# MLCogUP/nspeech

Hardware: AMD Instinct MI355X
Metric: mel-frames/sec Tacotron-2 LJSpeech bs32 train step (higher is better)
Workload: dtype bf16; 1 GPU; Tacotron-2 train step (fwd+bwd+clip+Adam), batch 32/GPU, T_in 160, T_out 1000, r=5; targets = spectrogram features of synthetic speech (SURVEY 8d); global_batch=32, parallelism=dp1, deterministic_gradients=True

## Files before the change

nspeech_amd/csrc/lstm_cluster.hip:

```cpp
#include "common.h"
#include <stdlib.h>
#include <stdint.h>

typedef unsigned long long u64;
constexpr int CW = 8;
constexpr int CTHREADS = CW * 64;

struct LstmClusterArgs {
  int N, T, H, P, padl, CS;
  const float* xg[2]; long ld_xg;
  const bf16_t* whT[2];
  const bf16_t* wh[2];
  bf16_t* h[2]; long ld_h;
  float* c[2];
  bf16_t* gates[2];
  const bf16_t* whT_hi[2]; const bf16_t* whT_lo[2];
  float* hf[2]; bf16_t* hb[2]; long ld_hb;
  const float* dh[2]; long ld_dh;
  bf16_t* dgates[2];
  const int* lengths;
  float forget_bias, cell_clip;
  u64* xbuf;
  int* status;
  int dbg;
  unsigned* flags;
  long long* trace;
};

__device__ __forceinline__ int swz_off(int row, int k, int H) {
  const int chunk = k >> 3;
  const int m = ((H >> 3) & 15) ? 7 : 15;
  return row * H + (((chunk ^ (row & m)) << 3) | (k & 7));
}

__global__ __launch_bounds__(CTHREADS) void lstm_cluster_fwd_kernel(LstmClusterArgs a) {
  extern __shared__ __attribute__((aligned(16))) char smem[];
  bf16_t* hs = (bf16_t*)smem;
  const int tid = threadIdx.x, lane = tid & 63, wave = tid >> 6;
  const int CS = a.CS, H = a.H;
  const int nrg = (a.N + 15) / 16;
  const int chain = blockIdx.x / CS, wgc = blockIdx.x % CS;
  const int d = chain / nrg, rg = chain % nrg;
  const int n0 = rg * 16;
  const int r16 = lane & 15, g = lane >> 4;
  const int GPR = H / 2;
  u64* xb = a.xbuf + (size_t)chain * 2 * 16 * GPR;
  const int uw0 = wgc * 64 + wave * 8;
  const int ksteps = H / 32;

  bf16x8 bw[2][16];
  {
    const bf16_t* W = a.whT[d];
    const int unit = uw0 + (r16 & 7);
#pragma unroll
    for (int tl = 0; tl < 2; ++tl) {
      const int gate = tl * 2 + (r16 >> 3);
      const bf16_t* row = W + ((long)gate * H + unit) * H;
#pragma unroll
      for (int ks = 0; ks < 16; ++ks)
        bw[tl][ks] = ks < ksteps ? *(const bf16x8*)(row + ks * 32 + g * 8) : (bf16x8){0, 0, 0, 0, 0, 0, 0, 0};
    }
  }
  float cst[4] = {0.f, 0.f, 0.f, 0.f};
  const bool cell_lane = r16 < 8;
  const int unit = uw0 + (r16 & 7);
  int len[4];
#pragma unroll
  for (int r = 0; r < 4; ++r) {
    const int n = n0 + g * 4 + r;
    len[r] = (a.lengths && n < a.N) ? a.lengths[n] : a.T;
  }
  const float* xg = a.xg[d];
  float xa[4], xb2[4], xa_n[4], xb_n[4];
  auto load_xg = [&](int t, float* pa, float* pb) {
#pragma unroll
    for (int r = 0; r < 4; ++r) {
      const int n = n0 + g * 4 + r;
      const long rowi = (long)n * a.P + a.padl + t;
      const bool ok = n < a.N;
      const int ga = (r16 >> 3), gb = 2 + (r16 >> 3);
      pa[r] = (ok && !(a.dbg & 1)) ? xg[rowi * a.ld_xg + (long)ga * H + unit] : 0.f;
      pb[r] = (ok && !(a.dbg & 1)) ? xg[rowi * a.ld_xg + (long)gb * H + unit] : 0.f;
    }
  };
  load_xg(d ? a.T - 1 : 0, xa, xb2);

  for (int step = 0; step < a.T; ++step) {
    const int t = d ? a.T - 1 - step : step;
    if (step + 1 < a.T) load_xg(d ? t - 1 : t + 1, xa_n, xb_n);
    f32x4 accA = {xa[0], xa[1], xa[2], xa[3]};
    f32x4 accB = {xb2[0], xb2[1], xb2[2], xb2[3]};
    if (step > 0) {
      const u64* cur = xb + (size_t)(step & 1) * 16 * GPR;
      const int total = 16 * GPR;
      for (int i0 = tid; i0 < total; i0 += CTHREADS * 4) {
        u64 v[4];
        unsigned spins = 0, clk0 = 0;
        bool ok;
        do {
          ok = true;
#pragma unroll
          for (int j = 0; j < 4; ++j) {
            const int i = i0 + j * CTHREADS;
            v[j] = i < total ? __hip_atomic_load(cur + i, __ATOMIC_RELAXED, __HIP_MEMORY_SCOPE_AGENT)
                             : ((u64)(unsigned)step << 32);
          }
#pragma unroll
          for (int j = 0; j < 4; ++j) ok = ok && ((unsigned)(v[j] >> 32) == (unsigned)step);
          if (a.dbg & 4) ok = true;
          if (!ok && (++spins & 1023u) == 0 && ns_spin_timed_out(clk0)) { atomicExch(a.status, 1); ok = true; }
        } while (!ok);
#pragma unroll
        for (int j = 0; j < 4; ++j) {
          const int i = i0 + j * CTHREADS;
          if (i < total) {
            const int row = i / GPR, pr = i % GPR;
            *(unsigned*)(hs + swz_off(row, pr * 2, H)) = (unsigned)v[j];
          }
        }
      }
      __syncthreads();
      if (*(volatile int*)a.status) return;
#pragma unroll
      for (int ks = 0; ks < 16; ++ks) {
        if (ks < ksteps) {
          const bf16x8 af = *(const bf16x8*)(hs + swz_off(r16, ks * 32 + g * 8, H));
          accA = __builtin_amdgcn_mfma_f32_16x16x32_bf16(af, bw[0][ks], accA, 0, 0, 0);
          accB = __builtin_amdgcn_mfma_f32_16x16x32_bf16(af, bw[1][ks], accB, 0, 0, 0);
        }
      }
      __syncthreads();
    }
    float hv[4], sgi[4], sgj[4], sgf[4], sgo[4];
#pragma unroll
    for (int r = 0; r < 4; ++r) {
      const float zj = __shfl_down(accA[r], 8, 64);
      const float zo = __shfl_down(accB[r], 8, 64);
      const bool masked = t >= len[r];
      const float gi = sigmoidf_(accA[r]), gj = tanhf_(zj), gf = sigmoidf_(accB[r] + a.forget_bias), go = sigmoidf_(zo);
      float cn = ns_cell_clip(gf * cst[r] + gi * gj, a.cell_clip);
      float hn = go * tanhf_(cn);
      if (masked) { cn = 0.f; hn = 0.f; }
      cst[r] = cn;
      hv[r] = hn;
      sgi[r] = masked ? 0.f : gi; sgj[r] = masked ? 0.f : gj; sgf[r] = masked ? 0.f : gf; sgo[r] = masked ? 0.f : go;
    }
    if (step + 1 < a.T) {
      u64* nxt = xb + (size_t)((step + 1) & 1) * 16 * GPR;
#pragma unroll
      for (int r = 0; r < 4; ++r) {
        const float hp = __shfl_down(hv[r], 1, 64);
        if (cell_lane && !(r16 & 1)) {
          const bf16_t b0 = (bf16_t)hv[r], b1 = (bf16_t)hp;
          const unsigned pay = (unsigned)(*(const unsigned short*)&b0) | ((unsigned)(*(const unsigned short*)&b1) << 16);
          const int row = g * 4 + r;
          __hip_atomic_store(nxt + (size_t)row * GPR + (unit >> 1), ((u64)(unsigned)(step + 1) << 32) | pay,
                             __ATOMIC_RELAXED, __HIP_MEMORY_SCOPE_AGENT);
        }
      }
    }
#pragma unroll
    for (int r = 0; r < 4; ++r) {
      const int n = n0 + g * 4 + r;
      if (cell_lane && n < a.N && !(a.dbg & 2)) {
        const long rowi = (long)n * a.P + a.padl + t;
        a.h[d][rowi * a.ld_h + unit] = (bf16_t)hv[r];
        a.c[d][rowi * H + unit] = cst[r];
        bf16_t* gp = a.gates[d] + rowi * 4 * H;
        gp[unit] = (bf16_t)sgi[r];
        gp[H + unit] = (bf16_t)sgj[r];
        gp[2 * H + unit] = (bf16_t)sgf[r];
        gp[3 * H + unit] = (bf16_t)sgo[r];
      }
    }
#pragma unroll
    for (int r = 0; r < 4; ++r) { xa[r] = xa_n[r]; xb2[r] = xb_n[r]; }
  }
}

__global__ __launch_bounds__(CTHREADS) void lstm_cluster_bwd_kernel(LstmClusterArgs a) {
  extern __shared__ __attribute__((aligned(16))) char smem[];
  const int CS = a.CS, H = a.H, K = 4 * a.H;
  bf16_t* dgs = (bf16_t*)smem;
  float* red = (float*)(smem + (size_t)16 * K * 2);
  const int tid = threadIdx.x, lane = tid & 63, wave = tid >> 6;
  const int nrg = (a.N + 15) / 16;
  const int chain = blockIdx.x / CS, wgc = blockIdx.x % CS;
  const int d = chain / nrg, rg = chain % nrg;
  const int n0 = rg * 16;
  const int r16 = lane & 15, g = lane >> 4;
  const int GPR = K / 2;
  u64* xb = a.xbuf + (size_t)chain * 2 * 16 * GPR;
  const int u0 = wgc * 64;
  const int kpw = K / CW;
  const int ksteps = kpw / 32;
  bf16x8 bw[4][8];
  {
    const bf16_t* W = a.wh[d];
#pragma unroll
    for (int tl = 0; tl < 4; ++tl) {
      const bf16_t* row = W + (long)(u0 + tl * 16 + r16) * K + wave * kpw;
#pragma unroll
      for (int ks = 0; ks < 8; ++ks)
        bw[tl][ks] = ks < ksteps ? *(const bf16x8*)(row + ks * 32 + g * 8) : (bf16x8){0, 0, 0, 0, 0, 0, 0, 0};
    }
  }
  const int er = tid >> 5, eu = (tid & 31) * 2;
  const int en = n0 + er;
  const int elen = (a.lengths && en < a.N) ? a.lengths[en] : a.T;
  float dcc[2] = {0.f, 0.f};

  for (int step = a.T - 1; step >= 0; --step) {
    const int t = d ? a.T - 1 - step : step;
    const int tp = d ? t + 1 : t - 1;
    const bool has_prev = step > 0;
    const bool has_next = step < a.T - 1;
    const int bs = a.T - 1 - step;
    float pdh[2] = {0.f, 0.f}, pg[2][4], pc[2] = {0.f, 0.f}, pcp[2] = {0.f, 0.f};
    const long rowi = (long)en * a.P + a.padl + t;
    const bool ok = en < a.N;
    const bool masked = t >= elen;
#pragma unroll
    for (int q = 0; q < 2; ++q) {
      const int u = u0 + eu + q;
#pragma unroll
      for (int j = 0; j < 4; ++j) pg[q][j] = ok ? (float)a.gates[d][rowi * 4 * H + (long)j * H + u] : 0.f;
      if (ok) {
        pdh[q] = a.dh[d][rowi * a.ld_dh + u];
        pc[q] = a.c[d][rowi * H + u];
        if (has_prev) pcp[q] = a.c[d][((long)en * a.P + a.padl + tp) * H + u];
      }
    }
    float dhp[2] = {0.f, 0.f};
    if (has_next) {
      const u64* cur = xb + (size_t)(bs & 1) * 16 * GPR;
      const int total = 16 * GPR;
      for (int i0 = tid; i0 < total; i0 += CTHREADS * 8) {
        u64 v[8];
        unsigned spins = 0, clk0 = 0;
        bool okk;
        do {
          okk = true;
#pragma unroll
          for (int j = 0; j < 8; ++j) {
            const int i = i0 + j * CTHREADS;
            v[j] = i < total ? __hip_atomic_load(cur + i, __ATOMIC_RELAXED, __HIP_MEMORY_SCOPE_AGENT)
                             : ((u64)(unsigned)bs << 32);
          }
#pragma unroll
          for (int j = 0; j < 8; ++j) okk = okk && ((unsigned)(v[j] >> 32) == (unsigned)bs);
          if (!okk && (++spins & 1023u) == 0 && ns_spin_timed_out(clk0)) { atomicExch(a.status, 2); okk = true; }
        } while (!okk);
#pragma unroll
        for (int j = 0; j < 8; ++j) {
          const int i = i0 + j * CTHREADS;
          if (i < total) {
            const int row = i / GPR, pr = i % GPR;
            *(unsigned*)(dgs + swz_off(row, pr * 2, K)) = (unsigned)v[j];
          }
        }
      }
      __syncthreads();
      if (*(volatile int*)a.status) return;
      f32x4 acc[4];
#pragma unroll
      for (int tl = 0; tl < 4; ++tl) acc[tl] = (f32x4){0.f, 0.f, 0.f, 0.f};
#pragma unroll
      for (int ks = 0; ks < 8; ++ks) {
        if (ks < ksteps) {
          const bf16x8 af = *(const bf16x8*)(dgs + swz_off(r16, wave * kpw + ks * 32 + g * 8, K));
#pragma unroll
          for (int tl = 0; tl < 4; ++tl) acc[tl] = __builtin_amdgcn_mfma_f32_16x16x32_bf16(af, bw[tl][ks], acc[tl], 0, 0, 0);
        }
      }
#pragma unroll
      for (int tl = 0; tl < 4; ++tl)
#pragma unroll
        for (int r = 0; r < 4; ++r) red[(wave * 16 + g * 4 + r) * 65 + tl * 16 + r16] = acc[tl][r];
      __syncthreads();
#pragma unroll
      for (int q = 0; q < 2; ++q) {
        float s = 0.f;
#pragma unroll
        for (int w = 0; w < CW; ++w) s += red[(w * 16 + er) * 65 + eu + q];
        dhp[q] = s;
      }
    }
    float dgv[2][4];
#pragma unroll
    for (int q = 0; q < 2; ++q) {
      const float gi = pg[q][0], gj = pg[q][1], gf = pg[q][2], go = pg[q][3];
      const float dh = pdh[q] + dhp[q];
      const float tc = tanhf_(pc[q]);
      const float d_o = dh * tc * go * (1.f - go);
      const float dc = dh * go * (1.f - tc * tc) + dcc[q];
      dgv[q][0] = dc * gj * gi * (1.f - gi);
      dgv[q][1] = dc * gi * (1.f - gj * gj);
      dgv[q][2] = dc * pcp[q] * gf * (1.f - gf);
      dgv[q][3] = d_o;
      dcc[q] = dc * gf;
      if (masked || !ok) {
        dgv[q][0] = dgv[q][1] = dgv[q][2] = dgv[q][3] = 0.f;
        dcc[q] = 0.f;
      }
    }
    if (step > 0) {
      u64* nxt = xb + (size_t)((bs + 1) & 1) * 16 * GPR;
#pragma unroll
      for (int j = 0; j < 4; ++j) {
        const bf16_t b0 = (bf16_t)dgv[0][j], b1 = (bf16_t)dgv[1][j];
        const unsigned pay = (unsigned)(*(const unsigned short*)&b0) | ((unsigned)(*(const unsigned short*)&b1) << 16);
        __hip_atomic_store(nxt + (size_t)er * GPR + ((j * H + u0 + eu) >> 1), ((u64)(unsigned)(bs + 1) << 32) | pay,
                           __ATOMIC_RELAXED, __HIP_MEMORY_SCOPE_AGENT);
      }
    }
    if (ok) {
#pragma unroll
      for (int j = 0; j < 4; ++j) {
        const bf16_t b0 = (bf16_t)dgv[0][j], b1 = (bf16_t)dgv[1][j];
        const unsigned pay = (unsigned)(*(const unsigned short*)&b0) | ((unsigned)(*(const unsigned short*)&b1) << 16);
        *(unsigned*)(a.dgates[d] + rowi * 4 * H + (long)j * H + u0 + eu) = pay;
      }
    }
    __syncthreads();
  }
}

constexpr int XW = 4;
constexpr int FW_POLL = 2;
constexpr int FW_WAVES = XW + 2 + FW_POLL;
constexpr int BW_POLL = 2;
constexpr int BW_WAVES = XW + 1 + BW_POLL + 1;
constexpr int XG_LD = 256 + 4;

__device__ __forceinline__ void wg_barrier() { asm volatile("s_waitcnt lgkmcnt(0)\n\ts_barrier" ::: "memory"); }
__device__ __forceinline__ unsigned pack_bf16(float lo, float hi) {
  const bf16_t b0 = (bf16_t)lo, b1 = (bf16_t)hi;
  return (unsigned)(*(const unsigned short*)&b0) | ((unsigned)(*(const unsigned short*)&b1) << 16);
}

template <int HB, int R>
__global__ __launch_bounds__(FW_WAVES * 64) void lstm_cluster2_fwd_kernel(LstmClusterArgs a) {
  extern __shared__ __attribute__((aligned(16))) char smem[];
  constexpr int H = HB * 64, KS = H / 32, CS = HB;
  constexpr int GPD = XW * 64 * 2;
  bf16_t* hs = (bf16_t*)smem;
  float* xgs = (float*)(smem + (size_t)2 * 16 * H * 2);
  constexpr int SV_H = 16 * 64 * 2, SV_C = 16 * 64 * 4, SV_G = 16 * 4 * 64 * 2, SV_BYTES = SV_H + SV_C + SV_G;
  char* svs = (char*)(xgs + 2 * 16 * XG_LD);
  int* abortf = (int*)(svs + 2 * SV_BYTES);
  const int tid = threadIdx.x, lane = tid & 63;
  const int wave = __builtin_amdgcn_readfirstlane(tid >> 6);
  const int nsets = ((a.N + 15) / 16 + R - 1) / R;
  const int set = blockIdx.x / CS, wgc = blockIdx.x % CS;
  const int d = set / nsets, rg0 = (set % nsets) * R;
  const int r16 = lane & 15, g = lane >> 4;
  u64* xb0 = a.xbuf + (size_t)(d * nsets * R + rg0) * 2 * CS * GPD;
  const int u0 = wgc * 64;
  const int T = a.T, Q = a.T * R;
  if (tid < 3) abortf[tid] = 0;

  if (wave < XW) {
    const int wq = wave * 16 + g * 4;
    bf16x8 bw[4][KS];
    {
      const bf16_t* W = a.whT[d];
#pragma unroll
      for (int gate = 0; gate < 4; ++gate) {
        const bf16_t* row = W + ((long)gate * H + u0 + wave * 16 + r16) * H;
#pragma unroll
        for (int ks = 0; ks < KS; ++ks) bw[gate][ks] = *(const bf16x8*)(row + ks * 32 + g * 8);
      }
    }
    float cst[R][4];
    int len[R];
    uint2 pend[R];
#pragma unroll
    for (int rg = 0; rg < R; ++rg) {
      const int n = (rg0 + rg) * 16 + r16;
      len[rg] = (a.lengths && n < a.N) ? a.lengths[n] : T;
      pend[rg] = make_uint2(0u, 0u);
#pragma unroll
      for (int r = 0; r < 4; ++r) cst[rg][r] = 0.f;
    }
    f32x4 acc[4];
    auto load_xg = [&](int q) {
      const float* xr = xgs + ((size_t)(q & 1) * 16 + r16) * XG_LD + wq;
#pragma unroll
      for (int gate = 0; gate < 4; ++gate) acc[gate] = *(const f32x4*)(xr + gate * 64);
    };
    wg_barrier();
    load_xg(0);
    for (int step = 0; step < T; ++step) {
      const int t = d ? T - 1 - step : step;
#pragma unroll
      for (int rg = 0; rg < R; ++rg) {
        const int q = step * R + rg, buf = q & 1;
        wg_barrier();
        if (abortf[buf]) return;
        const bool tr = (a.dbg & 16) && blockIdx.x == 0 && tid == 0 && q < 512;
        if (tr) a.trace[q * 8 + 0] = wall_clock64();
        if (R == 2 && q > 0)
          *(uint2*)(hs + (size_t)((q + 1) & 1) * 16 * H + swz_off(r16, u0 + wq, H)) = pend[(rg + 1) % R];
        if (step > 0) {
          const bf16_t* hb = hs + (size_t)buf * 16 * H;
#pragma unroll
          for (int ks = 0; ks < KS; ++ks) {
            const bf16x8 hf = *(const bf16x8*)(hb + swz_off(r16, ks * 32 + g * 8, H));
#pragma unroll
            for (int gate = 0; gate < 4; ++gate)
              acc[gate] = __builtin_amdgcn_mfma_f32_16x16x32_bf16(bw[gate][ks], hf, acc[gate], 0, 0, 0);
          }
        }
        const bool masked = t >= len[rg];
        float hv[4], sg[4][4];
#pragma unroll
        for (int r = 0; r < 4; ++r) {
          const float gi = sigmoidf_(acc[0][r]), gj = tanhf_(acc[1][r]);
          const float gf = sigmoidf_(acc[2][r] + a.forget_bias), go = sigmoidf_(acc[3][r]);
          float cn = ns_cell_clip(gf * cst[rg][r] + gi * gj, a.cell_clip);
          float hn = go * tanhf_(cn);
          if (masked) { cn = 0.f; hn = 0.f; }
          cst[rg][r] = cn;
          hv[r] = hn;
          sg[r][0] = masked ? 0.f : gi; sg[r][1] = masked ? 0.f : gj; sg[r][2] = masked ? 0.f : gf; sg[r][3] = masked ? 0.f : go;
        }
        if (tr) a.trace[q * 8 + 1] = wall_clock64();
        uint2 hp;
        hp.x = pack_bf16(hv[0], hv[1]);
        hp.y = pack_bf16(hv[2], hv[3]);
        if (step + 1 < T) {
          if (CS > 1) {
            u64* nxt = xb0 + ((size_t)rg * 2 + ((step + 1) & 1)) * CS * GPD + (size_t)wgc * GPD + (wave * 64 + lane) * 2;
            __hip_atomic_store(nxt, ((u64)(unsigned)(step + 1) << 32) | hp.x, __ATOMIC_RELAXED, __HIP_MEMORY_SCOPE_AGENT);
            __hip_atomic_store(nxt + 1, ((u64)(unsigned)(step + 1) << 32) | hp.y, __ATOMIC_RELAXED, __HIP_MEMORY_SCOPE_AGENT);
          }
          if (R == 1) *(uint2*)(hs + (size_t)((q + 1) & 1) * 16 * H + swz_off(r16, u0 + wq, H)) = hp;
          else pend[rg] = hp;
        }
        if (tr) a.trace[q * 8 + 2] = wall_clock64();
        {
          char* sv = svs + (size_t)buf * SV_BYTES;
          *(uint2*)((bf16_t*)sv + r16 * 64 + wq) = hp;
          *(f32x4*)((float*)(sv + SV_H) + r16 * 64 + wq) = (f32x4){cst[rg][0], cst[rg][1], cst[rg][2], cst[rg][3]};
          bf16_t* gp = (bf16_t*)(sv + SV_H + SV_C) + r16 * 4 * 64 + wq;
#pragma unroll
          for (int gate = 0; gate < 4; ++gate) {
            uint2 pk;
            pk.x = pack_bf16(sg[0][gate], sg[1][gate]);
            pk.y = pack_bf16(sg[2][gate], sg[3][gate]);
            *(uint2*)(gp + gate * 64) = pk;
          }
        }
        if (q + 1 < Q) load_xg(q + 1);
      }
    }
    wg_barrier();
  } else if (wave == XW || wave == XW + 3) {
    constexpr int NPG = (CS - 1) * GPD;
    constexpr int PPG = NPG / (FW_POLL * 64) > 0 ? NPG / (FW_POLL * 64) : 1;
    static_assert(CS == 1 || NPG == PPG * FW_POLL * 64, "poller coverage");
    const int j0 = (wave == XW ? 0 : 1) * PPG;
    wg_barrier();
    for (int q = 0; q < Q; ++q) {
      const int step = q / R, rg = q % R, buf = q & 1;
      const bool tr = (a.dbg & 16) && blockIdx.x == 0 && lane == 0 && wave == XW && q < 512;
      if (tr) a.trace[q * 8 + 4] = wall_clock64();
      if (step > 0 && CS > 1) {
        const u64* cur = xb0 + ((size_t)rg * 2 + (step & 1)) * CS * GPD;
        u64 v[PPG];
        unsigned spins = 0, clk0 = 0;
        bool ok;
        do {
          ok = true;
#pragma unroll
          for (int j = 0; j < PPG; ++j) {
            const int li = lane + 64 * (j0 + j), sx = li / GPD;
            const int ws = sx < wgc ? sx : sx + 1;
            v[j] = __hip_atomic_load(cur + (size_t)ws * GPD + (li % GPD), __ATOMIC_RELAXED, __HIP_MEMORY_SCOPE_AGENT);
          }
#pragma unroll
          for (int j = 0; j < PPG; ++j) ok = ok && ((unsigned)(v[j] >> 32) == (unsigned)step);
          if (!ok) {
            if ((++spins & 1023u) == 0) {
              if (__hip_atomic_load(a.status, __ATOMIC_RELAXED, __HIP_MEMORY_SCOPE_AGENT)) { abortf[buf] = 1; ok = true; }
              else if (ns_spin_timed_out(clk0)) { atomicExch(a.status, 1); abortf[buf] = 1; ok = true; }
            }
          }
        } while (!ok);
        if (tr) { a.trace[q * 8 + 5] = wall_clock64(); a.trace[q * 8 + 6] = spins; }
        bf16_t* dst = hs + (size_t)buf * 16 * H;
#pragma unroll
        for (int j = 0; j < PPG; ++j) {
          const int li = lane + 64 * (j0 + j), sx = li / GPD, lw = li % GPD;
          const int ws = sx < wgc ? sx : sx + 1;
          const int lp = (lw >> 1) & 63;
          const int k = ws * 64 + (lw >> 7) * 16 + (lp >> 4) * 4 + (lw & 1) * 2;
          *(unsigned*)(dst + swz_off(lp & 15, k, H)) = (unsigned)v[j];
        }
      }
      wg_barrier();
      if (abortf[buf]) return;
    }
    wg_barrier();
  } else if (wave == XW + 2) {
    auto save = [&](int q) {
      const int step = q / R, rg = q % R;
      const int t = d ? T - 1 - step : step;
      const int n0 = (rg0 + rg) * 16;
      const char* sv = svs + (size_t)(q & 1) * SV_BYTES;
#pragma unroll
      for (int j = 0; j < 14; ++j) {
        const int idx = lane + 64 * j;
        const f32x4 v = *(const f32x4*)(sv + idx * 16);
        if (idx < 128) {
          const int row = idx >> 3, cc = idx & 7;
          if (n0 + row < a.N)
            *(f32x4*)(a.h[d] + ((unsigned)((n0 + row) * a.P + a.padl + t) * (unsigned)a.ld_h + (unsigned)(u0 + cc * 8))) = v;
        } else if (idx < 384) {
          const int jj = idx - 128, row = jj >> 4, cc = jj & 15;
          if (n0 + row < a.N)
            *(f32x4*)(a.c[d] + ((unsigned)((n0 + row) * a.P + a.padl + t) * (unsigned)H + (unsigned)(u0 + cc * 4))) = v;
        } else {
          const int jj = idx - 384, row = jj >> 5, gate = (jj >> 3) & 3, cc = jj & 7;
          if (n0 + row < a.N)
            *(f32x4*)(a.gates[d] + ((unsigned)((n0 + row) * a.P + a.padl + t) * (unsigned)(4 * H) + (unsigned)(gate * H + u0 + cc * 8))) = v;
        }
      }
    };
    wg_barrier();
    for (int q = 0; q < Q; ++q) {
      wg_barrier();
      if (abortf[q & 1]) return;
      if (q > 0) save(q - 1);
    }
    wg_barrier();
    save(Q - 1);
  } else {
    f32x4 pf[16];
    const float* xg = a.xg[d];
    const int pgate = lane >> 4, pf4 = (lane & 15) * 4;
    auto pf_load = [&](int q) {
      const int step = q / R, rg = q % R;
      const int t = d ? T - 1 - step : step;
      const int n0 = (rg0 + rg) * 16;
#pragma unroll
      for (int j = 0; j < 16; ++j) {
        const int n = n0 + j;
        pf[j] = n < a.N ? *(const f32x4*)(xg + ((unsigned)(n * a.P + a.padl + t) * (unsigned)a.ld_xg + (unsigned)(pgate * H + u0 + pf4)))
                        : (f32x4){0.f, 0.f, 0.f, 0.f};
      }
    };
    auto pf_store = [&](int buf) {
#pragma unroll
      for (int j = 0; j < 16; ++j) *(f32x4*)(xgs + ((size_t)buf * 16 + j) * XG_LD + pgate * 64 + pf4) = pf[j];
    };
    pf_load(0);
    pf_store(0);
    if (Q > 1) pf_load(1);
    wg_barrier();
    for (int q = 0; q < Q; ++q) {
      if (q + 1 < Q) {
        pf_store((q + 1) & 1);
        if (q + 2 < Q) pf_load(q + 2);
      }
      wg_barrier();
      if (abortf[q & 1]) return;
    }
    wg_barrier();
  }
}


constexpr int X3W = 4, X3_POLL = 2, X3_UPW = 32;
constexpr int X3_WAVES = X3W + X3_POLL + 2;
constexpr int XG3_LD = 4 * X3_UPW + 4;

template <int HB, int R>
__global__ __launch_bounds__(X3_WAVES * 64) void lstm_cluster3_fwd_kernel(LstmClusterArgs a) {
  extern __shared__ __attribute__((aligned(16))) char smem[];
  constexpr int H = HB * 64, KS = H / 32, GPC = 16 * H;
  constexpr int CS = H / X3_UPW;
  constexpr int PPG = GPC / (X3_POLL * 64);
  static_assert(GPC % (X3_POLL * 64) == 0, "poller coverage");
  bf16_t* hsh = (bf16_t*)smem;
  bf16_t* hsl = hsh + 2 * 16 * H;
  float* xgs = (float*)(hsl + 2 * 16 * H);
  constexpr int SV_H = 16 * 32 * 4, SV_C = 16 * 32 * 4, SV_G = 16 * 4 * 32 * 2, SV_HB = 16 * 32 * 2;
  constexpr int SV_BYTES = SV_H + SV_C + SV_G + SV_HB;
  char* svs = (char*)(xgs + 2 * 16 * XG3_LD);
  int* abortf = (int*)(svs + 2 * SV_BYTES);
  const int tid = threadIdx.x, lane = tid & 63;
  const int wave = __builtin_amdgcn_readfirstlane(tid >> 6);
  const int nsets = ((a.N + 15) / 16 + R - 1) / R;
  const int set = blockIdx.x / CS, wgc = blockIdx.x % CS;
  const int d = set / nsets, rg0 = (set % nsets) * R;
  const int r16 = lane & 15, g = lane >> 4;
  u64* xb0 = a.xbuf + (size_t)(d * nsets * R + rg0) * 2 * GPC;
  const int u0 = wgc * X3_UPW;
  const int T = a.T, Q = a.T * R;
  if (tid < 2) abortf[tid] = 0;

  if (wave < X3W) {
    const int ul = wave * 8 + (r16 & 7);
    const bool cell_lane = r16 < 8;
    const int pub0 = (((wgc * X3W + wave) * 32) + g * 8 + (r16 & 7)) * 4;
    bf16x8 bwh[2][KS], bwl[2][KS];
    {
#pragma unroll
      for (int tl = 0; tl < 2; ++tl) {
        const int gate = tl * 2 + (r16 >> 3);
        const long wrow = ((long)gate * H + u0 + ul) * H + g * 8;
#pragma unroll
        for (int ks = 0; ks < KS; ++ks) {
          bwh[tl][ks] = *(const bf16x8*)(a.whT_hi[d] + wrow + ks * 32);
          bwl[tl][ks] = *(const bf16x8*)(a.whT_lo[d] + wrow + ks * 32);
        }
      }
    }
    float cst[R][4];
    int len[R][4];
#pragma unroll
    for (int rg = 0; rg < R; ++rg)
#pragma unroll
      for (int r = 0; r < 4; ++r) {
        const int n = (rg0 + rg) * 16 + g * 4 + r;
        cst[rg][r] = 0.f;
        len[rg][r] = (a.lengths && n < a.N) ? a.lengths[n] : T;
      }
    for (int step = 0; step < T; ++step) {
      const int t = d ? T - 1 - step : step;
#pragma unroll
      for (int rg = 0; rg < R; ++rg) {
        const int q = step * R + rg, buf = q & 1;
        wg_barrier();
        if (abortf[buf]) return;
        const float* xr = xgs + (size_t)buf * 16 * XG3_LD + (r16 >> 3) * X3_UPW + ul;
        f32x4 accA, accB;
#pragma unroll
        for (int r = 0; r < 4; ++r) {
          accA[r] = xr[(g * 4 + r) * XG3_LD];
          accB[r] = xr[(g * 4 + r) * XG3_LD + 2 * X3_UPW];
        }
        if (step > 0) {
          const bf16_t* hbh = hsh + (size_t)buf * 16 * H;
          const bf16_t* hbl = hsl + (size_t)buf * 16 * H;
#pragma unroll
          for (int ks = 0; ks < KS; ++ks) {
            const int so = swz_off(r16, ks * 32 + g * 8, H);
            const bf16x8 ah = *(const bf16x8*)(hbh + so), al = *(const bf16x8*)(hbl + so);
            accA = mfma_split<3>(ah, al, bwh[0][ks], bwl[0][ks], accA);
            accB = mfma_split<3>(ah, al, bwh[1][ks], bwl[1][ks], accB);
          }
        }
        float hv[4], sg[4][4], cn4[4];
#pragma unroll
        for (int r = 0; r < 4; ++r) {
          const float zj = __shfl_down(accA[r], 8, 64), zo = __shfl_down(accB[r], 8, 64);
          const bool masked = t >= len[rg][r];
          const float gi = sigmoidf_(accA[r]), gj = tanhf_(zj), gf = sigmoidf_(accB[r] + a.forget_bias), go = sigmoidf_(zo);
          float cn = ns_cell_clip(gf * cst[rg][r] + gi * gj, a.cell_clip);
          float hn = go * tanhf_(cn);
          if (masked) { cn = 0.f; hn = 0.f; }
          cst[rg][r] = cn;
          cn4[r] = cn;
          hv[r] = hn;
          sg[r][0] = masked ? 0.f : gi; sg[r][1] = masked ? 0.f : gj; sg[r][2] = masked ? 0.f : gf; sg[r][3] = masked ? 0.f : go;
        }
        if (step + 1 < T && cell_lane) {
          u64* nxt = xb0 + ((size_t)rg * 2 + ((step + 1) & 1)) * GPC + pub0;
#pragma unroll
          for (int r = 0; r < 4; ++r)
            __hip_atomic_store(nxt + r, ((u64)(unsigned)(step + 1) << 32) | (u64)__float_as_uint(hv[r]), __ATOMIC_RELAXED,
                               __HIP_MEMORY_SCOPE_AGENT);
        }
        if (cell_lane) {
          char* sv = svs + (size_t)buf * SV_BYTES;
#pragma unroll
          for (int r = 0; r < 4; ++r) {
            const int row = g * 4 + r;
            ((float*)sv)[row * X3_UPW + ul] = hv[r];
            ((float*)(sv + SV_H))[row * X3_UPW + ul] = cn4[r];
            bf16_t* gp = (bf16_t*)(sv + SV_H + SV_C) + row * 4 * X3_UPW + ul;
#pragma unroll
            for (int gate = 0; gate < 4; ++gate) gp[gate * X3_UPW] = (bf16_t)sg[r][gate];
            ((bf16_t*)(sv + SV_H + SV_C + SV_G))[row * X3_UPW + ul] = (bf16_t)hv[r];
          }
        }
      }
    }
    wg_barrier();
  } else if (wave < X3W + X3_POLL) {
    const int j0 = (wave - X3W) * PPG;
    const int pr_ = lane & 3, pu = (lane >> 2) & 7, pgl = lane >> 5;
    for (int q = 0; q < Q; ++q) {
      const int step = q / R, rg = q % R, buf = q & 1;
      if (step > 0) {
        const u64* cur = xb0 + ((size_t)rg * 2 + (step & 1)) * GPC;
        u64 v[PPG];
        unsigned spins = 0, clk0 = 0;
        bool ok;
        do {
          ok = true;
#pragma unroll
          for (int j = 0; j < PPG; ++j) v[j] = __hip_atomic_load(cur + lane + (j0 + j) * 64, __ATOMIC_RELAXED, __HIP_MEMORY_SCOPE_AGENT);
#pragma unroll
          for (int j = 0; j < PPG; ++j) ok = ok && ((unsigned)(v[j] >> 32) == (unsigned)step);
          if (!ok) {
            if ((++spins & 1023u) == 0) {
              if (__hip_atomic_load(a.status, __ATOMIC_RELAXED, __HIP_MEMORY_SCOPE_AGENT)) { abortf[buf] = 1; ok = true; }
              else if (ns_spin_timed_out(clk0)) { atomicExch(a.status, 1); abortf[buf] = 1; ok = true; }
            }
          }
        } while (!ok);
        bf16_t* dh_ = hsh + (size_t)buf * 16 * H;
        bf16_t* dl_ = hsl + (size_t)buf * 16 * H;
#pragma unroll
        for (int j = 0; j < PPG; ++j) {
          const int jj = j0 + j;
          const int row = (((jj & 1) << 1) | pgl) * 4 + pr_;
          const int k = (jj >> 3) * X3_UPW + ((jj >> 1) & 3) * 8 + pu;
          const float x = __uint_as_float((unsigned)v[j]);
          const bf16_t hi = (bf16_t)x;
          const int so = swz_off(row, k, H);
          dh_[so] = hi;
          dl_[so] = (bf16_t)(x - (float)hi);
        }
      }
      wg_barrier();
      if (abortf[buf]) return;
    }
    wg_barrier();
  } else if (wave == X3W + X3_POLL) {
    auto save = [&](int q) {
      const int step = q / R, rg = q % R;
      const int t = d ? T - 1 - step : step;
      const int n0 = (rg0 + rg) * 16;
      const char* sv = svs + (size_t)(q & 1) * SV_BYTES;
#pragma unroll
      for (int j = 0; j < 9; ++j) {
        const int idx = lane + 64 * j;
        const f32x4 v = *(const f32x4*)(sv + idx * 16);
        if (idx < 128) {
          const int row = idx >> 3, cc = idx & 7;
          if (n0 + row < a.N)
            *(f32x4*)(a.hf[d] + ((unsigned)((n0 + row) * a.P + a.padl + t) * (unsigned)a.ld_h + (unsigned)(u0 + cc * 4))) = v;
        } else if (idx < 256) {
          const int jj = idx - 128, row = jj >> 3, cc = jj & 7;
          if (n0 + row < a.N)
            *(f32x4*)(a.c[d] + ((unsigned)((n0 + row) * a.P + a.padl + t) * (unsigned)H + (unsigned)(u0 + cc * 4))) = v;
        } else if (idx < 512) {
          const int jj = idx - 256, row = jj >> 4, gate = (jj >> 2) & 3, cc = jj & 3;
          if (n0 + row < a.N)
            *(f32x4*)(a.gates[d] + ((unsigned)((n0 + row) * a.P + a.padl + t) * (unsigned)(4 * H) + (unsigned)(gate * H + u0 + cc * 8))) = v;
        } else {
          const int jj = idx - 512, row = jj >> 2, cc = jj & 3;
          if (a.hb[d] && n0 + row < a.N)
            *(f32x4*)(a.hb[d] + ((unsigned)((n0 + row) * a.P + a.padl + t) * (unsigned)a.ld_hb + (unsigned)(u0 + cc * 8))) = v;
        }
      }
    };
    for (int q = 0; q < Q; ++q) {
      wg_barrier();
      if (abortf[q & 1]) return;
      if (q > 0) save(q - 1);
    }
    wg_barrier();
    save(Q - 1);
  } else {
    f32x4 pf[8];
    const float* xg = a.xg[d];
    const int prow = lane >> 5, pgate = (lane >> 3) & 3, pf4 = (lane & 7) * 4;
    auto pf_load = [&](int q) {
      const int step = q / R, rg = q % R;
      const int t = d ? T - 1 - step : step;
      const int n0 = (rg0 + rg) * 16;
#pragma unroll
      for (int j = 0; j < 8; ++j) {
        const int n = n0 + 2 * j + prow;
        pf[j] = n < a.N ? *(const f32x4*)(xg + ((unsigned)(n * a.P + a.padl + t) * (unsigned)a.ld_xg + (unsigned)(pgate * H + u0 + pf4)))
                        : (f32x4){0.f, 0.f, 0.f, 0.f};
      }
    };
    auto pf_store = [&](int buf) {
#pragma unroll
      for (int j = 0; j < 8; ++j) *(f32x4*)(xgs + ((size_t)buf * 16 + 2 * j + prow) * XG3_LD + pgate * X3_UPW + pf4) = pf[j];
    };
    pf_load(0);
    pf_store(0);
    if (Q > 1) pf_load(1);
    for (int q = 0; q < Q; ++q) {
      wg_barrier();
      if (abortf[q & 1]) return;
      if (q + 1 < Q) {
        pf_store((q + 1) & 1);
        if (q + 2 < Q) pf_load(q + 2);
      }
    }
    wg_barrier();
  }
}

typedef unsigned int u32x4 __attribute__((ext_vector_type(4)));

template <int HB, int R>
__global__ __launch_bounds__(BW_WAVES * 64) void lstm_cluster2_bwd_kernel(LstmClusterArgs a) {
  extern __shared__ __attribute__((aligned(16))) char smem[];
  constexpr int H = HB * 64, K = 4 * H, KS = K / 32;
  constexpr int CPL = K / 64;
  const int CS = HB;
  bf16_t* dgs = (bf16_t*)smem;
  char* ops = smem + (size_t)2 * 16 * K * 2;
  constexpr int OPS_STAGE = 16 * 4 * 64 * 2 + 2 * 16 * 64 * 4;
  bf16_t* outs = (bf16_t*)(ops + 2 * OPS_STAGE);
  float* c0 = (float*)(outs + 2 * 16 * 4 * 64);
  int* abortf = (int*)(c0 + R * 16 * 64);
  int* ready = abortf + 2;
  const int tid = threadIdx.x, lane = tid & 63;
  const int wave = __builtin_amdgcn_readfirstlane(tid >> 6);
  const int nsets = ((a.N + 15) / 16 + R - 1) / R;
  const int set = blockIdx.x / CS, wgc = blockIdx.x % CS;
  const int d = set / nsets, rg0 = (set % nsets) * R;
  const int r16 = lane & 15, g = lane >> 4;
  unsigned* flags0 = a.flags + (size_t)(d * nsets * R + rg0) * 8;
  const int u0 = wgc * 64;
  const int T = a.T, Q = a.T * R;
  if (tid < 3) abortf[tid] = 0;
  auto t_of = [&](int step) { return d ? T - 1 - step : step; };

  if (wave < XW) {
    const int wu = wave * 16 + r16;
    bf16x8 bw[KS];
    {
      const bf16_t* row = a.wh[d] + (long)(u0 + wu) * K;
#pragma unroll
      for (int ks = 0; ks < KS; ++ks) bw[ks] = *(const bf16x8*)(row + ks * 32 + g * 8);
    }
    int asw[4];
#pragma unroll
    for (int m = 0; m < 4; ++m) asw[m] = r16 * K + (((m * 4 + g) ^ r16) << 3);
    float dcc[R][4], pc[R][4];
    int len[R][4];
#pragma unroll
    for (int rg = 0; rg < R; ++rg)
#pragma unroll
      for (int r = 0; r < 4; ++r) {
        const int n = (rg0 + rg) * 16 + g * 4 + r;
        dcc[rg][r] = 0.f; pc[rg][r] = 0.f;
        len[rg][r] = (a.lengths && n < a.N) ? a.lengths[n] : T;
      }
    for (int bs = 0; bs < T; ++bs) {
      const int t = t_of(T - 1 - bs);
#pragma unroll
      for (int rg = 0; rg < R; ++rg) {
        const int q = bs * R + rg, buf = q & 1;
        const int n0 = (rg0 + rg) * 16;
        wg_barrier();
        if (abortf[buf]) return;
        f32x4 acc = {0.f, 0.f, 0.f, 0.f};
        if (bs > 0) {
          const bf16_t* db = dgs + (size_t)buf * 16 * K;
          f32x4 acc2 = {0.f, 0.f, 0.f, 0.f};
#pragma unroll
          for (int ks = 0; ks < KS; ks += 2) {
            const bf16x8 a0 = *(const bf16x8*)(db + asw[ks & 3] + (ks >> 2) * 128);
            const bf16x8 a1 = *(const bf16x8*)(db + asw[(ks + 1) & 3] + ((ks + 1) >> 2) * 128);
            acc = __builtin_amdgcn_mfma_f32_16x16x32_bf16(a0, bw[ks], acc, 0, 0, 0);
            acc2 = __builtin_amdgcn_mfma_f32_16x16x32_bf16(a1, bw[ks + 1], acc2, 0, 0, 0);
          }
#pragma unroll
          for (int r = 0; r < 4; ++r) acc[r] += acc2[r];
        }
        const char* st = ops + (size_t)buf * OPS_STAGE;
        const bf16_t* sgt = (const bf16_t*)st;
        const float* sdh = (const float*)(st + 8192);
        const float* scp = (const float*)(st + 12288);
        bf16_t* so = outs + (size_t)buf * 16 * 4 * 64;
#pragma unroll
        for (int r = 0; r < 4; ++r) {
          const int row = g * 4 + r;
          const int n = n0 + row;
          const float gi = (float)sgt[(row * 4 + 0) * 64 + wu], gj = (float)sgt[(row * 4 + 1) * 64 + wu];
          const float gf = (float)sgt[(row * 4 + 2) * 64 + wu], go = (float)sgt[(row * 4 + 3) * 64 + wu];
          const float cprev = scp[row * 64 + wu];
          const float ccur = bs == 0 ? c0[(rg * 16 + row) * 64 + wu] : pc[rg][r];
          const float dh = sdh[row * 64 + wu] + acc[r];
          const float tc = tanhf_(ccur);
          const float d_o = dh * tc * go * (1.f - go);
          const float dc = dh * go * (1.f - tc * tc) + dcc[rg][r];
          float dgv[4] = {dc * gj * gi * (1.f - gi), dc * gi * (1.f - gj * gj), dc * cprev * gf * (1.f - gf), d_o};
          dcc[rg][r] = dc * gf;
          if (t >= len[rg][r] || n >= a.N) {
            dgv[0] = dgv[1] = dgv[2] = dgv[3] = 0.f;
            dcc[rg][r] = 0.f;
          }
          pc[rg][r] = cprev;
#pragma unroll
          for (int j = 0; j < 4; ++j) so[(row * 4 + j) * 64 + wu] = (bf16_t)dgv[j];
        }
        if (lane == 0) __hip_atomic_fetch_add(ready, 1, __ATOMIC_RELEASE, __HIP_MEMORY_SCOPE_WORKGROUP);
      }
    }
    wg_barrier();
  } else if (wave == XW) {
    const long dg_bytes = (long)a.N * a.P * K * 2;
    const auto rsrc = __builtin_amdgcn_make_buffer_rsrc((void*)a.dgates[d], 0, (int)dg_bytes, 0x00020000);
    wg_barrier();
    for (int q = 0; q < Q; ++q) {
      const int bs = q / R, rg = q % R;
      const int t = t_of(T - 1 - bs);
      const int n0 = (rg0 + rg) * 16;
      unsigned spins = 0, clk0 = 0;
      while (__hip_atomic_load(ready, __ATOMIC_ACQUIRE, __HIP_MEMORY_SCOPE_WORKGROUP) < XW * (q + 1)) {
        __builtin_amdgcn_s_sleep(1);
        if (((++spins) & 255) == 0) {
          if (abortf[0] | abortf[1]) return;
          if ((spins & 1023u) == 0 && ns_spin_timed_out(clk0)) { atomicExch(a.status, 3); return; }
        }
      }
      const char* so = (const char*)(outs + (size_t)(q & 1) * 16 * 4 * 64);
#pragma unroll
      for (int j = 0; j < 8; ++j) {
        const int idx = lane + 64 * j, c8 = idx & 7, gate = (idx >> 3) & 3, row = idx >> 5;
        const u32x4 v = *(const u32x4*)(so + idx * 16);
        if (n0 + row < a.N) {
          const unsigned off = ((unsigned)((n0 + row) * a.P + a.padl + t) * (unsigned)K + (unsigned)(gate * H + u0 + c8 * 8)) * 2u;
          __builtin_amdgcn_raw_buffer_store_b128(v, rsrc, off, 0, 16);
        }
      }
      if (R > 1) wg_barrier();
      if (bs + 1 < T) {
        asm volatile("s_waitcnt vmcnt(0)" ::: "memory");
        if (lane == 0) __hip_atomic_store(flags0 + rg * 8 + wgc, (unsigned)(bs + 1), __ATOMIC_RELAXED, __HIP_MEMORY_SCOPE_AGENT);
      }
      if (R == 1) wg_barrier();
    }
  } else if (wave < XW + 1 + BW_POLL) {
    const int pl = (wave - XW - 1) * 64 + lane;
    const long dg_bytes = (long)a.N * a.P * K * 2;
    const auto rsrc = __builtin_amdgcn_make_buffer_rsrc((void*)a.dgates[d], 0, (int)dg_bytes, 0x00020000);
    for (int q = 0; q < Q; ++q) {
      const int bs = q / R, rg = q % R, buf = q & 1;
      if (bs > 0) {
        const unsigned* fl = flags0 + rg * 8;
        unsigned spins = 0, clk0 = 0;
        for (;;) {
          const unsigned v = lane < CS ? __hip_atomic_load(fl + lane, __ATOMIC_RELAXED, __HIP_MEMORY_SCOPE_AGENT) : 0xffffffffu;
          if (__all(v >= (unsigned)bs)) break;
          if ((++spins & 1023u) == 0) {
            if (__hip_atomic_load(a.status, __ATOMIC_RELAXED, __HIP_MEMORY_SCOPE_AGENT)) { abortf[buf] = 1; break; }
            if (ns_spin_timed_out(clk0)) { atomicExch(a.status, 2); abortf[buf] = 1; break; }
          }
        }
        const int tn = t_of(T - bs);
        const int n0 = (rg0 + rg) * 16;
        bf16_t* dst = dgs + (size_t)buf * 16 * K;
        u32x4 v[CPL];
#pragma unroll
        for (int j = 0; j < CPL; ++j) {
          const int idx = pl + 128 * j, row = idx / (K / 8), ch = idx % (K / 8);
          v[j] = (u32x4){0u, 0u, 0u, 0u};
          if (n0 + row < a.N) {
            const unsigned off = ((unsigned)((n0 + row) * a.P + a.padl + tn) * (unsigned)K + (unsigned)(ch * 8)) * 2u;
            v[j] = __builtin_amdgcn_raw_buffer_load_b128(rsrc, off, 0, 16);
          }
        }
#pragma unroll
        for (int j = 0; j < CPL; ++j) {
          const int idx = pl + 128 * j, row = idx / (K / 8), ch = idx % (K / 8);
          *(u32x4*)(dst + swz_off(row, ch * 8, K)) = v[j];
        }
      }
      wg_barrier();
      if (abortf[buf]) return;
    }
    wg_barrier();
  } else {
    f32x4 pg[8], pd[4], pcp[4];
    auto pf_load = [&](int q) {
      const int bs = q / R, rg = q % R, step = T - 1 - bs;
      const int t = t_of(step), tp = d ? t + 1 : t - 1;
      const bool has_prev = step > 0;
      const int n0 = (rg0 + rg) * 16;
#pragma unroll
      for (int j = 0; j < 8; ++j) {
        const int idx = lane + 64 * j, c8 = idx & 7, gate = (idx >> 3) & 3, row = idx >> 5;
        const int n = n0 + row;
        pg[j] = n < a.N ? *(const f32x4*)(a.gates[d] + ((unsigned)(n * a.P + a.padl + t) * (unsigned)(4 * H) + (unsigned)(gate * H + u0 + c8 * 8)))
                        : (f32x4){0.f, 0.f, 0.f, 0.f};
      }
#pragma unroll
      for (int j = 0; j < 4; ++j) {
        const int idx = lane + 64 * j, c16 = idx & 15, row = idx >> 4;
        const int n = n0 + row;
        pd[j] = n < a.N ? *(const f32x4*)(a.dh[d] + ((unsigned)(n * a.P + a.padl + t) * (unsigned)a.ld_dh + (unsigned)(u0 + c16 * 4)))
                        : (f32x4){0.f, 0.f, 0.f, 0.f};
        pcp[j] = (n < a.N && has_prev) ? *(const f32x4*)(a.c[d] + ((unsigned)(n * a.P + a.padl + tp) * (unsigned)H + (unsigned)(u0 + c16 * 4)))
                                       : (f32x4){0.f, 0.f, 0.f, 0.f};
      }
    };
    auto pf_store = [&](int buf) {
      char* st = ops + (size_t)buf * OPS_STAGE;
#pragma unroll
      for (int j = 0; j < 8; ++j) *(f32x4*)(st + (size_t)(lane + 64 * j) * 16) = pg[j];
#pragma unroll
      for (int j = 0; j < 4; ++j) {
        *(f32x4*)(st + 8192 + (size_t)(lane + 64 * j) * 16) = pd[j];
        *(f32x4*)(st + 12288 + (size_t)(lane + 64 * j) * 16) = pcp[j];
      }
    };
    {
      const int t0 = t_of(T - 1);
#pragma unroll
      for (int rg = 0; rg < R; ++rg)
#pragma unroll
        for (int j = 0; j < 4; ++j) {
          const int idx = lane + 64 * j, c16 = idx & 15, row = idx >> 4;
          const int n = (rg0 + rg) * 16 + row;
          const f32x4 v = n < a.N ? *(const f32x4*)(a.c[d] + ((unsigned)(n * a.P + a.padl + t0) * (unsigned)H + (unsigned)(u0 + c16 * 4)))
                                  : (f32x4){0.f, 0.f, 0.f, 0.f};
          *(f32x4*)(c0 + (rg * 16 * 64) + idx * 4) = v;
        }
      pf_load(0);
      pf_store(0);
      if (Q > 1) pf_load(1);
    }
    for (int q = 0; q < Q; ++q) {
      wg_barrier();
      if (abortf[q & 1]) return;
      if (q + 1 < Q) {
        pf_store((q + 1) & 1);
        if (q + 2 < Q) pf_load(q + 2);
      }
    }
    wg_barrier();
  }
}


constexpr int BP_WAVES = XW + 2;
constexpr int DGI_LD = 256 + 8;

template <int HB, int R>
__global__ __launch_bounds__(BP_WAVES * 64) void lstm_cluster2p_bwd_kernel(LstmClusterArgs a) {
  extern __shared__ __attribute__((aligned(16))) char smem[];
  constexpr int H = HB * 64, K4 = 4 * H, CS = HB;
  constexpr int GPD = 16 * 32;
  bf16_t* dgi = (bf16_t*)smem;
  char* ops = (char*)(dgi + 2 * 16 * DGI_LD);
  constexpr int OPS_G = 16 * 4 * 64 * 2, OPS_F = 16 * 64 * 4;
  constexpr int OPS_STAGE = OPS_G + 2 * OPS_F;
  float* c0 = (float*)(ops + 2 * OPS_STAGE);
  int* abortf = (int*)(c0 + R * 16 * 64);
  const int tid = threadIdx.x, lane = tid & 63;
  const int wave = __builtin_amdgcn_readfirstlane(tid >> 6);
  const int nsets = ((a.N + 15) / 16 + R - 1) / R;
  const int set = blockIdx.x / CS, wgc = blockIdx.x % CS;
  const int d = set / nsets, rg0 = (set % nsets) * R;
  const int r16 = lane & 15, g = lane >> 4;
  u64* xb0 = a.xbuf + (size_t)(d * nsets * R + rg0) * 2 * CS * CS * GPD;
  const int u0 = wgc * 64;
  const int T = a.T, Q = a.T * R;
  if (tid == 0) abortf[0] = 0;
  auto t_of = [&](int step) { return d ? T - 1 - step : step; };

  if (wave < XW) {
    const int wu = wave * 16 + r16;
    bf16x8 bw[HB][8];
#pragma unroll
    for (int j = 0; j < HB; ++j) {
      const bf16_t* row = a.wh[d] + (long)(j * 64 + wu) * K4 + u0;
#pragma unroll
      for (int ks = 0; ks < 8; ++ks)
#pragma unroll
        for (int e = 0; e < 8; ++e) bw[j][ks][e] = row[(e & 3) * H + ks * 8 + g * 2 + (e >> 2)];
    }
    float dcc[R][4], pc[R][4];
    f32x4 ownp[R];
    int len[R][4];
#pragma unroll
    for (int rg = 0; rg < R; ++rg) {
      ownp[rg] = (f32x4){0.f, 0.f, 0.f, 0.f};
#pragma unroll
      for (int r = 0; r < 4; ++r) {
        const int n = (rg0 + rg) * 16 + g * 4 + r;
        dcc[rg][r] = 0.f; pc[rg][r] = 0.f;
        len[rg][r] = (a.lengths && n < a.N) ? a.lengths[n] : T;
      }
    }
    float kdo[4], kdc[4], ki[4], kj[4], kf[4], dhx[4], cpv[4], gfv[4];
    auto indep = [&](int q) {
      const int bs = q / R, rg = q % R;
      const char* st = ops + (size_t)(q & 1) * OPS_STAGE;
      const bf16_t* sgt = (const bf16_t*)st;
      const float* sdh = (const float*)(st + OPS_G);
      const float* scp = (const float*)(st + OPS_G + OPS_F);
#pragma unroll
      for (int r = 0; r < 4; ++r) {
        const int row = g * 4 + r;
        const float gi = (float)sgt[(row * 4 + 0) * 64 + wu], gj = (float)sgt[(row * 4 + 1) * 64 + wu];
        const float gf = (float)sgt[(row * 4 + 2) * 64 + wu], go = (float)sgt[(row * 4 + 3) * 64 + wu];
        const float cprev = scp[row * 64 + wu];
        float ccur = c0[(rg * 16 + row) * 64 + wu];
        if (bs > 0) ccur = R == 1 ? pc[0][r] : (rg ? pc[R - 1][r] : pc[0][r]);
        const float tc = tanhf_(ccur);
        dhx[r] = sdh[row * 64 + wu];
        kdo[r] = tc * go * (1.f - go);
        kdc[r] = go * (1.f - tc * tc);
        ki[r] = gj * gi * (1.f - gi);
        kj[r] = gi * (1.f - gj * gj);
        kf[r] = cprev * gf * (1.f - gf);
        cpv[r] = cprev; gfv[r] = gf;
      }
    };
    wg_barrier();
    indep(0);
    for (int bs = 0; bs < T; ++bs) {
      const int t = t_of(T - 1 - bs);
#pragma unroll
      for (int rg = 0; rg < R; ++rg) {
        const int q = bs * R + rg, buf = q & 1;
        const int n0 = (rg0 + rg) * 16;
        const bool tr = (a.dbg & 16) && blockIdx.x == 0 && tid == 0 && q < 512;
        if (tr) a.trace[q * 8 + 0] = wall_clock64();
        f32x4 rec = ownp[rg];
        if (bs > 0 && CS > 1) {
          const u64* cur = xb0 + ((size_t)rg * 2 + (bs & 1)) * CS * CS * GPD + (size_t)wgc * CS * GPD + (g * 2) * 64 + wu;
          u64 v[CS > 1 ? CS - 1 : 1][2];
          unsigned spins = 0, clk0 = 0;
          bool ok;
          do {
            ok = true;
#pragma unroll
            for (int sx = 0; sx < CS - 1; ++sx) {
              const int ws = sx < wgc ? sx : sx + 1;
#pragma unroll
              for (int h = 0; h < 2; ++h) v[sx][h] = __hip_atomic_load(cur + (size_t)ws * GPD + h * 64, __ATOMIC_RELAXED, __HIP_MEMORY_SCOPE_AGENT);
            }
#pragma unroll
            for (int sx = 0; sx < CS - 1; ++sx)
#pragma unroll
              for (int h = 0; h < 2; ++h) ok = ok && ((unsigned)(v[sx][h] >> 32) == (unsigned)bs);
            if (!ok && (++spins & 1023u) == 0) {
              if (__hip_atomic_load(a.status, __ATOMIC_RELAXED, __HIP_MEMORY_SCOPE_AGENT)) { abortf[0] = 1; ok = true; }
              else if (ns_spin_timed_out(clk0)) { atomicExch(a.status, 2); abortf[0] = 1; ok = true; }
            }
          } while (!ok);
          if (tr) { a.trace[q * 8 + 4] = wall_clock64(); a.trace[q * 8 + 6] = spins; }
#pragma unroll
          for (int sx = 0; sx < CS - 1; ++sx)
#pragma unroll
            for (int h = 0; h < 2; ++h) {
              const unsigned pay = (unsigned)v[sx][h];
              rec[2 * h] += __uint_as_float(pay << 16);
              rec[2 * h + 1] += __uint_as_float(pay & 0xffff0000u);
            }
        }
        bf16_t* di = dgi + (size_t)buf * 16 * DGI_LD;
#pragma unroll
        for (int r = 0; r < 4; ++r) {
          const int row = g * 4 + r;
          const int n = n0 + row;
          const float dh = dhx[r] + rec[r];
          const float d_o = dh * kdo[r];
          const float dc = dh * kdc[r] + dcc[rg][r];
          float dgv[4] = {dc * ki[r], dc * kj[r], dc * kf[r], d_o};
          dcc[rg][r] = dc * gfv[r];
          if (t >= len[rg][r] || n >= a.N) {
            dgv[0] = dgv[1] = dgv[2] = dgv[3] = 0.f;
            dcc[rg][r] = 0.f;
          }
          pc[rg][r] = cpv[r];
          uint2 pk;
          pk.x = pack_bf16(dgv[0], dgv[1]);
          pk.y = pack_bf16(dgv[2], dgv[3]);
          *(uint2*)(di + row * DGI_LD + wu * 4) = pk;
        }
        if (tr) a.trace[q * 8 + 1] = wall_clock64();
        wg_barrier();
        if (abortf[0]) return;
        if (tr) a.trace[q * 8 + 2] = wall_clock64();
        if (bs + 1 < T) {
          f32x4 acc[HB];
#pragma unroll
          for (int j = 0; j < HB; ++j) acc[j] = (f32x4){0.f, 0.f, 0.f, 0.f};
#pragma unroll
          for (int ks = 0; ks < 8; ++ks) {
            const bf16x8 af = *(const bf16x8*)(di + r16 * DGI_LD + ks * 32 + g * 8);
#pragma unroll
            for (int j = 0; j < HB; ++j) acc[j] = __builtin_amdgcn_mfma_f32_16x16x32_bf16(af, bw[j][ks], acc[j], 0, 0, 0);
          }
          indep(q + 1);
          if (tr) a.trace[q * 8 + 3] = wall_clock64();
          u64* nxt = xb0 + ((size_t)rg * 2 + ((bs + 1) & 1)) * CS * CS * GPD;
#pragma unroll
          for (int j = 0; j < HB; ++j) {
            if (j == wgc) {
              ownp[rg] = acc[j];
            } else {
              u64* dst = nxt + (size_t)(j * CS + wgc) * GPD + (g * 2) * 64 + wu;
#pragma unroll
              for (int h = 0; h < 2; ++h)
                __hip_atomic_store(dst + h * 64, ((u64)(unsigned)(bs + 1) << 32) | pack_bf16(acc[j][2 * h], acc[j][2 * h + 1]),
                                   __ATOMIC_RELAXED, __HIP_MEMORY_SCOPE_AGENT);
            }
          }
          if (tr) a.trace[q * 8 + 7] = wall_clock64();
        } else if (q + 1 < Q) {
          indep(q + 1);
        }
      }
    }
  } else if (wave == XW) {
    auto save = [&](int q) {
      const int bs = q / R, rg = q % R;
      const int t = t_of(T - 1 - bs);
      const int n0 = (rg0 + rg) * 16;
      const bf16_t* di = dgi + (size_t)(q & 1) * 16 * DGI_LD;
#pragma unroll
      for (int jj = 0; jj < 2; ++jj) {
        const int idx = lane + 64 * jj, c8 = idx & 7, row = idx >> 3;
        uint2 x[8];
#pragma unroll
        for (int e = 0; e < 8; ++e) x[e] = *(const uint2*)(di + row * DGI_LD + (c8 * 8 + e) * 4);
        if (n0 + row < a.N) {
          bf16_t* out = a.dgates[d] + ((unsigned)((n0 + row) * a.P + a.padl + t) * (unsigned)K4 + (unsigned)(u0 + c8 * 8));
#pragma unroll
          for (int gate = 0; gate < 4; ++gate) {
            unsigned w[4];
#pragma unroll
            for (int e2 = 0; e2 < 4; ++e2) {
              const unsigned lo = gate < 2 ? x[2 * e2].x : x[2 * e2].y, hi = gate < 2 ? x[2 * e2 + 1].x : x[2 * e2 + 1].y;
              w[e2] = (gate & 1) ? ((lo >> 16) | (hi & 0xffff0000u)) : ((lo & 0xffffu) | (hi << 16));
            }
            *(uint4*)(out + gate * H) = make_uint4(w[0], w[1], w[2], w[3]);
          }
        }
      }
    };
    wg_barrier();
    for (int q = 0; q < Q; ++q) {
      if (q > 0) save(q - 1);
      wg_barrier();
      if (abortf[0]) return;
    }
    save(Q - 1);
  } else {
    f32x4 pg[8], pd[4], pcp[4];
    auto pf_load = [&](int q) {
      const int bs = q / R, rg = q % R, step = T - 1 - bs;
      const int t = t_of(step), tp = d ? t + 1 : t - 1;
      const bool has_prev = step > 0;
      const int n0 = (rg0 + rg) * 16;
#pragma unroll
      for (int j = 0; j < 8; ++j) {
        const int idx = lane + 64 * j, c8 = idx & 7, gate = (idx >> 3) & 3, row = idx >> 5;
        const int n = n0 + row;
        pg[j] = n < a.N ? *(const f32x4*)(a.gates[d] + ((unsigned)(n * a.P + a.padl + t) * (unsigned)(4 * H) + (unsigned)(gate * H + u0 + c8 * 8)))
                        : (f32x4){0.f, 0.f, 0.f, 0.f};
      }
#pragma unroll
      for (int j = 0; j < 4; ++j) {
        const int idx = lane + 64 * j, c16 = idx & 15, row = idx >> 4;
        const int n = n0 + row;
        pd[j] = n < a.N ? *(const f32x4*)(a.dh[d] + ((unsigned)(n * a.P + a.padl + t) * (unsigned)a.ld_dh + (unsigned)(u0 + c16 * 4)))
                        : (f32x4){0.f, 0.f, 0.f, 0.f};
        pcp[j] = (n < a.N && has_prev) ? *(const f32x4*)(a.c[d] + ((unsigned)(n * a.P + a.padl + tp) * (unsigned)H + (unsigned)(u0 + c16 * 4)))
                                       : (f32x4){0.f, 0.f, 0.f, 0.f};
      }
    };
    auto pf_store = [&](int buf) {
      char* st = ops + (size_t)buf * OPS_STAGE;
#pragma unroll
      for (int j = 0; j < 8; ++j) *(f32x4*)(st + (size_t)(lane + 64 * j) * 16) = pg[j];
#pragma unroll
      for (int j = 0; j < 4; ++j) {
        *(f32x4*)(st + OPS_G + (size_t)(lane + 64 * j) * 16) = pd[j];
        *(f32x4*)(st + OPS_G + OPS_F + (size_t)(lane + 64 * j) * 16) = pcp[j];
      }
    };
    {
      const int t0 = t_of(T - 1);
#pragma unroll
      for (int rg = 0; rg < R; ++rg)
#pragma unroll
        for (int j = 0; j < 4; ++j) {
          const int idx = lane + 64 * j, c16 = idx & 15, row = idx >> 4;
          const int n = (rg0 + rg) * 16 + row;
          const f32x4 v = n < a.N ? *(const f32x4*)(a.c[d] + ((unsigned)(n * a.P + a.padl + t0) * (unsigned)H + (unsigned)(u0 + c16 * 4)))
                                  : (f32x4){0.f, 0.f, 0.f, 0.f};
          *(f32x4*)(c0 + (rg * 16 * 64) + idx * 4) = v;
        }
      pf_load(0);
      pf_store(0);
      if (Q > 1) pf_load(1);
    }
    wg_barrier();
    for (int q = 0; q < Q; ++q) {
      if (q + 1 < Q) {
        pf_store((q + 1) & 1);
        if (q + 2 < Q) pf_load(q + 2);
      }
      wg_barrier();
      if (abortf[0]) return;
    }
  }
}

static int cluster_supported(const ns_lstm_seq_params* p0, const ns_lstm_seq_params* p1) {
  return p0->dtype == NS_BF16 && p1->dtype == NS_BF16 && p0->H % 64 == 0 && p0->H <= 512 && p0->T >= 2;
}
static int cluster3_supported(const ns_lstm_seq_params* p0, const ns_lstm_seq_params* p1) {
  auto al16 = [](const void* p) { return ((uintptr_t)p & 15) == 0; };
  const ns_lstm_seq_params* pp[2] = {p0, p1};
  if (p0->H % 64 != 0 || p0->H > 256 || p0->T < 2 || p0->N < 1) return 0;
  if (2 * ((p0->N + 15) / 16 + 1) * 8 * sizeof(unsigned) > 4096) return 0;
  for (int d = 0; d < 2; ++d) {
    const ns_lstm_seq_params* p = pp[d];
    if (p->dtype != NS_F32 || p->f32_passes != 3 || !p->whT_hi || !p->whT_lo || !p->xg || !p->h || !p->c || !p->gates) return 0;
    if (!(al16(p->xg) && p->ld_xg % 4 == 0 && al16(p->h) && p->ld_h % 4 == 0 && al16(p->c) && al16(p->gates) &&
          al16(p->whT_hi) && al16(p->whT_lo))) return 0;
    if (p->h_bf16 && !(al16(p->h_bf16) && p->ld_h_bf16 % 8 == 0)) return 0;
    const long widest = p->ld_xg > 4L * p->H ? p->ld_xg : 4L * p->H;
    if ((long)p->N * p->P * widest >= (1L << 31)) return 0;
  }
  return 1;
}
extern "C" int ns_lstm_cluster_supported(const ns_lstm_seq_params* p0, const ns_lstm_seq_params* p1, int backward) {
  if (!p0 || !p1) return 0;
  if (!(p0->reverse == 0 && p1->reverse == 1 && p0->N == p1->N && p0->T == p1->T && p0->H == p1->H)) return 0;
  if ((p0->H + 31) / 32 > ns_device_cus()) return 0;
  if (cluster_supported(p0, p1)) return 1;
  return !backward && cluster3_supported(p0, p1);
}

extern "C" size_t ns_lstm_cluster_work_bytes(const ns_lstm_seq_params* p) {
  if (!p) return 0;
  const size_t chains = 2 * (size_t)((p->N + 15) / 16 + 1);
  return chains * 2 * 16 * (size_t)(4 * p->H / 2) * sizeof(u64) + 256 + 4096 + 512 * 8 * sizeof(long long);
}

constexpr size_t FLAG_BYTES = 4096;
static void fill(LstmClusterArgs& a, const ns_lstm_seq_params* p0, const ns_lstm_seq_params* p1, void* work) {
  const ns_lstm_seq_params* pp[2] = {p0, p1};
  a.N = p0->N; a.T = p0->T; a.H = p0->H; a.P = p0->P; a.padl = p0->padl; a.CS = p0->H / 64;
  a.ld_xg = p0->ld_xg; a.ld_h = p0->ld_h; a.ld_dh = p0->ld_dh;
  a.lengths = p0->lengths; a.forget_bias = p0->forget_bias; a.cell_clip = p0->cell_clip;
  for (int d = 0; d < 2; ++d) {
    a.xg[d] = pp[d]->xg; a.whT[d] = (const bf16_t*)pp[d]->whT; a.wh[d] = (const bf16_t*)pp[d]->wh;
    a.h[d] = (bf16_t*)pp[d]->h; a.c[d] = pp[d]->c; a.gates[d] = (bf16_t*)pp[d]->gates;
    a.dh[d] = pp[d]->dh; a.dgates[d] = (bf16_t*)pp[d]->dgates;
    a.whT_hi[d] = (const bf16_t*)pp[d]->whT_hi; a.whT_lo[d] = (const bf16_t*)pp[d]->whT_lo;
    a.hf[d] = (float*)pp[d]->h; a.hb[d] = (bf16_t*)pp[d]->h_bf16;
  }
  a.ld_hb = p0->ld_h_bf16;
  a.status = (int*)work;
  a.flags = (unsigned*)((char*)work + 256);
  a.xbuf = (u64*)((char*)work + 256 + FLAG_BYTES);
  const char* dbg = getenv("NS_CLUSTER_DBG");
  a.dbg = dbg ? atoi(dbg) : 0;
  const size_t chains = 2 * (size_t)((a.N + 15) / 16 + 1);
  a.trace = (long long*)((char*)work + 256 + FLAG_BYTES + chains * 2 * 16 * (size_t)(4 * a.H / 2) * sizeof(u64));
}

static bool role_split_ok(const LstmClusterArgs& a, bool bwd) {
  if (a.dbg & 8) return false;
  if (a.H > 256 || a.H % 64) return false;
  if (2 * ((a.N + 15) / 16 + 1) * 8 * sizeof(unsigned) > FLAG_BYTES) return false;
  const long widest = a.ld_xg > 4L * a.H ? a.ld_xg : 4L * a.H;
  if ((long)a.N * a.P * (widest > a.ld_dh ? widest : a.ld_dh) >= (1L << 31)) return false;
  auto al16 = [](const void* p) { return ((uintptr_t)p & 15) == 0; };
  for (int d = 0; d < 2; ++d) {
    if (!bwd && !(al16(a.xg[d]) && a.ld_xg % 4 == 0 && al16(a.h[d]) && a.ld_h % 8 == 0 && al16(a.c[d]) && al16(a.gates[d]))) return false;
    if (bwd && !(al16(a.dh[d]) && a.ld_dh % 4 == 0 && al16(a.c[d]) && al16(a.gates[d]) && al16(a.dgates[d]))) return false;
  }
  return true;
}

extern "C" int ns_lstm_cluster_fwd(const ns_lstm_seq_params* p0, const ns_lstm_seq_params* p1, void* work,
                                   ns_stream_t s_) {
  hipStream_t s = (hipStream_t)s_;
  NS_CHECK_ARG(p0 && p1 && work, "ns_lstm_cluster_fwd: null");
  if (p0->dtype != NS_F32) NS_CHECK_ARG(cluster_supported(p0, p1), "ns_lstm_cluster_fwd: needs bf16, H %% 64 == 0, H <= 512, T >= 2");
  NS_CHECK_ARG(p0->reverse == 0 && p1->reverse == 1 && p0->N == p1->N && p0->T == p1->T && p0->H == p1->H,
               "ns_lstm_cluster_fwd: p0 forward / p1 reversed with equal shapes expected");
  if (p0->dtype == NS_F32) {
    NS_CHECK_ARG(cluster3_supported(p0, p1), "ns_lstm_cluster_fwd: the fp32 form needs H %% 64 == 0, H <= 256, T >= 2, "
                 "f32_passes 3 with whT_hi / whT_lo, 16-byte aligned operands");
    LstmClusterArgs a = {};
    fill(a, p0, p1, work);
    const int nrg = (a.N + 15) / 16, R = (nrg >= 2 && (a.dbg & 1024)) ? 2 : 1;
    const size_t xbytes = (2 * (size_t)nrg + 2) * 2 * 16 * (size_t)a.H * sizeof(u64);
    { const int zrc = ns_zero_async(work, ((256 + FLAG_BYTES + xbytes) + 15) & ~(size_t)15, s); if (zrc) return zrc; }
    const size_t lds3 = (size_t)2 * 2 * 16 * a.H * 2 + sizeof(float) * 2 * 16 * XG3_LD + 2 * 9216 + 32;
    const dim3 grid((unsigned)(2 * ((nrg + R - 1) / R) * (a.H / X3_UPW))), block(X3_WAVES * 64);
#define NS_LAUNCH_F3(HB_) \
    do { \
      static bool attr3 = false; \
      if (!attr3) { \
        (void)hipFuncSetAttribute((const void*)lstm_cluster3_fwd_kernel<HB_, 2>, hipFuncAttributeMaxDynamicSharedMemorySize, 160 * 1024); \
        (void)hipFuncSetAttribute((const void*)lstm_cluster3_fwd_kernel<HB_, 1>, hipFuncAttributeMaxDynamicSharedMemorySize, 160 * 1024); \
        attr3 = true; \
      } \
      if (R == 2) hipLaunchKernelGGL((lstm_cluster3_fwd_kernel<HB_, 2>), grid, block, lds3, s, a); \
      else hipLaunchKernelGGL((lstm_cluster3_fwd_kernel<HB_, 1>), grid, block, lds3, s, a); \
    } while (0)
    switch (a.H / 64) {
      case 1: NS_LAUNCH_F3(1); break;
      case 2: NS_LAUNCH_F3(2); break;
      case 3: NS_LAUNCH_F3(3); break;
      default: NS_LAUNCH_F3(4); break;
    }
#undef NS_LAUNCH_F3
    NS_CHECK_LAUNCH("lstm_cluster3_fwd");
    return NS_OK;
  }
  NS_CHECK_ARG(cluster_supported(p0, p1), "ns_lstm_cluster_fwd: needs bf16, H %% 64 == 0, H <= 512, T >= 2");
  LstmClusterArgs a = {};
  fill(a, p0, p1, work);
  const size_t chains = 2 * (size_t)((a.N + 15) / 16);
  const size_t xbytes = (chains + 2) * 2 * 16 * (size_t)(a.H / 2) * sizeof(u64);
  { const int zrc = ns_zero_async(work, ((256 + FLAG_BYTES + xbytes) + 15) & ~(size_t)15, s); if (zrc) return zrc; }
  if (role_split_ok(a, false)) {
    const size_t lds2 = (size_t)2 * 16 * a.H * 2 + sizeof(float) * 2 * 16 * XG_LD + 2 * (2048 + 4096 + 8192) + 32;
    const int nrg = (a.N + 15) / 16, R = (nrg >= 2 && (a.dbg & 512)) ? 2 : 1;
    const dim3 grid((unsigned)(2 * ((nrg + R - 1) / R) * a.CS)), block(FW_WAVES * 64);
#define NS_LAUNCH_F(HB_) \
    if (R == 2) hipLaunchKernelGGL((lstm_cluster2_fwd_kernel<HB_, 2>), grid, block, lds2, s, a); \
    else hipLaunchKernelGGL((lstm_cluster2_fwd_kernel<HB_, 1>), grid, block, lds2, s, a)
    switch (a.H / 64) {
      case 1: NS_LAUNCH_F(1); break;
      case 2: NS_LAUNCH_F(2); break;
      case 3: NS_LAUNCH_F(3); break;
      default: NS_LAUNCH_F(4); break;
    }
#undef NS_LAUNCH_F
    NS_CHECK_LAUNCH("lstm_cluster2_fwd");
    return NS_OK;
  }
  const size_t lds = (size_t)16 * a.H * 2;
  hipLaunchKernelGGL(lstm_cluster_fwd_kernel, dim3((unsigned)(chains * a.CS)), dim3(CTHREADS), lds, s, a);
  NS_CHECK_LAUNCH("lstm_cluster_fwd");
  return NS_OK;
}

extern "C" int ns_lstm_cluster_bwd(const ns_lstm_seq_params* p0, const ns_lstm_seq_params* p1, void* work,
                                   ns_stream_t s_) {
  hipStream_t s = (hipStream_t)s_;
  NS_CHECK_ARG(p0 && p1 && work, "ns_lstm_cluster_bwd: null");
  NS_CHECK_ARG(cluster_supported(p0, p1), "ns_lstm_cluster_bwd: needs bf16, H %% 64 == 0, H <= 512, T >= 2");
  NS_CHECK_ARG(p0->reverse == 0 && p1->reverse == 1 && p0->N == p1->N && p0->T == p1->T && p0->H == p1->H,
               "ns_lstm_cluster_bwd: p0 forward / p1 reversed with equal shapes expected");
  LstmClusterArgs a = {};
  fill(a, p0, p1, work);
  const size_t chains = 2 * (size_t)((a.N + 15) / 16);
  const size_t xbytes = role_split_ok(a, true)
                            ? ((a.dbg & 64) ? 0 : (chains + 2) * 2 * (size_t)a.CS * a.CS * 512 * sizeof(u64))
                            : (chains + 2) * 2 * 16 * (size_t)(4 * a.H / 2) * sizeof(u64);
  { const int zrc = ns_zero_async(work, ((256 + FLAG_BYTES + xbytes) + 15) & ~(size_t)15, s); if (zrc) return zrc; }
  static bool attr = false;
  if (!attr) {
    (void)hipFuncSetAttribute((const void*)lstm_cluster_bwd_kernel, hipFuncAttributeMaxDynamicSharedMemorySize, 160 * 1024);
    (void)hipFuncSetAttribute((const void*)lstm_cluster2_bwd_kernel<3, 1>, hipFuncAttributeMaxDynamicSharedMemorySize, 160 * 1024);
    (void)hipFuncSetAttribute((const void*)lstm_cluster2_bwd_kernel<4, 1>, hipFuncAttributeMaxDynamicSharedMemorySize, 160 * 1024);
    (void)hipFuncSetAttribute((const void*)lstm_cluster2_bwd_kernel<2, 2>, hipFuncAttributeMaxDynamicSharedMemorySize, 160 * 1024);
    (void)hipFuncSetAttribute((const void*)lstm_cluster2_bwd_kernel<3, 2>, hipFuncAttributeMaxDynamicSharedMemorySize, 160 * 1024);
    (void)hipFuncSetAttribute((const void*)lstm_cluster2_bwd_kernel<4, 2>, hipFuncAttributeMaxDynamicSharedMemorySize, 160 * 1024);
    attr = true;
  }
  if (role_split_ok(a, true) && !(a.dbg & 64)) {
    const int nrg = (a.N + 15) / 16, R = (nrg >= 2 && (a.dbg & 2048)) ? 2 : 1;
    const int CS = a.CS;
    const size_t ldsp = (size_t)2 * 16 * DGI_LD * 2 + 2 * 16384 + sizeof(float) * (size_t)R * 16 * 64 + 32;
    const dim3 grid((unsigned)(2 * ((nrg + R - 1) / R) * CS)), block(BP_WAVES * 64);
#define NS_LAUNCH_BP(HB_) \
    do { \
      if (R == 2) hipLaunchKernelGGL((lstm_cluster2p_bwd_kernel<HB_, 2>), grid, block, ldsp, s, a); \
      else hipLaunchKernelGGL((lstm_cluster2p_bwd_kernel<HB_, 1>), grid, block, ldsp, s, a); \
    } while (0)
    switch (a.H / 64) {
      case 1: NS_LAUNCH_BP(1); break;
      case 2: NS_LAUNCH_BP(2); break;
      case 3: NS_LAUNCH_BP(3); break;
      default: NS_LAUNCH_BP(4); break;
    }
#undef NS_LAUNCH_BP
    NS_CHECK_LAUNCH("lstm_cluster2p_bwd");
    return NS_OK;
  }
  if (role_split_ok(a, true)) {
    const int nrg = (a.N + 15) / 16, R = (nrg >= 3 && !(a.dbg & 32)) ? 2 : 1;
    const size_t lds2 = (size_t)2 * 16 * 4 * a.H * 2 + 2 * 16384 + 2 * 8192 + (size_t)R * 4096 + 32;
    const dim3 grid((unsigned)(2 * ((nrg + R - 1) / R) * a.CS)), block(BW_WAVES * 64);
#define NS_LAUNCH_B(HB_) \
    if (R == 2) hipLaunchKernelGGL((lstm_cluster2_bwd_kernel<HB_, 2>), grid, block, lds2, s, a); \
    else hipLaunchKernelGGL((lstm_cluster2_bwd_kernel<HB_, 1>), grid, block, lds2, s, a)
    switch (a.H / 64) {
      case 1: NS_LAUNCH_B(1); break;
      case 2: NS_LAUNCH_B(2); break;
      case 3: NS_LAUNCH_B(3); break;
      default: NS_LAUNCH_B(4); break;
    }
#undef NS_LAUNCH_B
    NS_CHECK_LAUNCH("lstm_cluster2_bwd");
    return NS_OK;
  }
  const size_t lds = (size_t)16 * 4 * a.H * 2 + sizeof(float) * CW * 16 * 65;
  hipLaunchKernelGGL(lstm_cluster_bwd_kernel, dim3((unsigned)(chains * a.CS)), dim3(CTHREADS), lds, s, a);
  NS_CHECK_LAUNCH("lstm_cluster_bwd");
  return NS_OK;
}
```

Measured before the change: 1.590 million mel-frames/s.

## Split LSTM cluster chains into fewer batch rows to spread across more CUs

Adds a rows-per-chain template parameter (16, 8 or 4) to the clustered LSTM forward and backward kernels, so a chain can cover fewer batch rows. The host picks the smallest row count whose grid still fits in half the CUs, unless overridden by an environment variable. With batch 32 this yields more independent chains, raising parallelism across CUs for the latency-bound recurrence. The cost is more workgroups, more cross-workgroup exchange traffic, idle lanes inside the 16-row MFMA tiles, and added LDS zeroing at kernel start.

```diff
diff --git a/nspeech_amd/csrc/lstm_cluster.hip b/nspeech_amd/csrc/lstm_cluster.hip
--- a/nspeech_amd/csrc/lstm_cluster.hip
+++ b/nspeech_amd/csrc/lstm_cluster.hip
@@ -339,19 +339,20 @@
   return (unsigned)(*(const unsigned short*)&b0) | ((unsigned)(*(const unsigned short*)&b1) << 16);
 }
 
-template <int HB, int R>
+template <int HB, int R, int RPC>
 __global__ __launch_bounds__(FW_WAVES * 64) void lstm_cluster2_fwd_kernel(LstmClusterArgs a) {
   extern __shared__ __attribute__((aligned(16))) char smem[];
   constexpr int H = HB * 64, KS = H / 32, CS = HB;
-  constexpr int GPD = XW * 64 * 2;
+  static_assert(RPC == 16 || ((RPC == 8 || RPC == 4) && R == 1), "rows per chain");
+  constexpr int GPD = XW * (4 * RPC) * 2;
   bf16_t* hs = (bf16_t*)smem;
   float* xgs = (float*)(smem + (size_t)2 * 16 * H * 2);
-  constexpr int SV_H = 16 * 64 * 2, SV_C = 16 * 64 * 4, SV_G = 16 * 4 * 64 * 2, SV_BYTES = SV_H + SV_C + SV_G;
+  constexpr int SV_H = RPC * 64 * 2, SV_C = RPC * 64 * 4, SV_G = RPC * 4 * 64 * 2, SV_BYTES = SV_H + SV_C + SV_G;
   char* svs = (char*)(xgs + 2 * 16 * XG_LD);
   int* abortf = (int*)(svs + 2 * SV_BYTES);
   const int tid = threadIdx.x, lane = tid & 63;
   const int wave = __builtin_amdgcn_readfirstlane(tid >> 6);
-  const int nsets = ((a.N + 15) / 16 + R - 1) / R;
+  const int nsets = ((a.N + RPC - 1) / RPC + R - 1) / R;
   const int set = blockIdx.x / CS, wgc = blockIdx.x % CS;
   const int d = set / nsets, rg0 = (set % nsets) * R;
   const int r16 = lane & 15, g = lane >> 4;
@@ -359,8 +360,13 @@
   const int u0 = wgc * 64;
   const int T = a.T, Q = a.T * R;
   if (tid < 3) abortf[tid] = 0;
+  if (RPC < 16) {
+    for (int i = tid; i < 2 * 16 * H / 8; i += FW_WAVES * 64) ((uint4*)hs)[i] = make_uint4(0u, 0u, 0u, 0u);
+    if (blockIdx.x == 0 && tid == 0) a.status[1] = RPC;
+  }
 
   if (wave < XW) {
+    const bool live = RPC == 16 || r16 < RPC;
     const int wq = wave * 16 + g * 4;
     bf16x8 bw[4][KS];
     {
@@ -377,8 +383,8 @@
     uint2 pend[R];
 #pragma unroll
     for (int rg = 0; rg < R; ++rg) {
-      const int n = (rg0 + rg) * 16 + r16;
-      len[rg] = (a.lengths && n < a.N) ? a.lengths[n] : T;
+      const int n = (rg0 + rg) * RPC + r16;
+      len[rg] = (a.lengths && live && n < a.N) ? a.lengths[n] : T;
       pend[rg] = make_uint2(0u, 0u);
 #pragma unroll
       for (int r = 0; r < 4; ++r) cst[rg][r] = 0.f;
@@ -430,16 +436,16 @@
         hp.x = pack_bf16(hv[0], hv[1]);
         hp.y = pack_bf16(hv[2], hv[3]);
         if (step + 1 < T) {
-          if (CS > 1) {
-            u64* nxt = xb0 + ((size_t)rg * 2 + ((step + 1) & 1)) * CS * GPD + (size_t)wgc * GPD + (wave * 64 + lane) * 2;
+          if (CS > 1 && live) {
+            u64* nxt = xb0 + ((size_t)rg * 2 + ((step + 1) & 1)) * CS * GPD + (size_t)wgc * GPD + (wave * 4 * RPC + g * RPC + r16) * 2;
             __hip_atomic_store(nxt, ((u64)(unsigned)(step + 1) << 32) | hp.x, __ATOMIC_RELAXED, __HIP_MEMORY_SCOPE_AGENT);
             __hip_atomic_store(nxt + 1, ((u64)(unsigned)(step + 1) << 32) | hp.y, __ATOMIC_RELAXED, __HIP_MEMORY_SCOPE_AGENT);
           }
-          if (R == 1) *(uint2*)(hs + (size_t)((q + 1) & 1) * 16 * H + swz_off(r16, u0 + wq, H)) = hp;
+          if (R == 1) { if (live) *(uint2*)(hs + (size_t)((q + 1) & 1) * 16 * H + swz_off(r16, u0 + wq, H)) = hp; }
           else pend[rg] = hp;
         }
         if (tr) a.trace[q * 8 + 2] = wall_clock64();
-        {
+        if (live) {
           char* sv = svs + (size_t)buf * SV_BYTES;
           *(uint2*)((bf16_t*)sv + r16 * 64 + wq) = hp;
           *(f32x4*)((float*)(sv + SV_H) + r16 * 64 + wq) = (f32x4){cst[rg][0], cst[rg][1], cst[rg][2], cst[rg][3]};
@@ -494,9 +500,9 @@
         for (int j = 0; j < PPG; ++j) {
           const int li = lane + 64 * (j0 + j), sx = li / GPD, lw = li % GPD;
           const int ws = sx < wgc ? sx : sx + 1;
-          const int lp = (lw >> 1) & 63;
-          const int k = ws * 64 + (lw >> 7) * 16 + (lp >> 4) * 4 + (lw & 1) * 2;
-          *(unsigned*)(dst + swz_off(lp & 15, k, H)) = (unsigned)v[j];
+          const int lp = (lw >> 1) % (4 * RPC);
+          const int k = ws * 64 + (lw / (8 * RPC)) * 16 + (lp / RPC) * 4 + (lw & 1) * 2;
+          *(unsigned*)(dst + swz_off(lp % RPC, k, H)) = (unsigned)v[j];
         }
       }
       wg_barrier();
@@ -504,25 +510,27 @@
     }
     wg_barrier();
   } else if (wave == XW + 2) {
+    constexpr int NH = RPC * 8, NC = RPC * 16, NG = RPC * 32, NJ = (NH + NC + NG + 63) / 64;
     auto save = [&](int q) {
       const int step = q / R, rg = q % R;
       const int t = d ? T - 1 - step : step;
-      const int n0 = (rg0 + rg) * 16;
+      const int n0 = (rg0 + rg) * RPC;
       const char* sv = svs + (size_t)(q & 1) * SV_BYTES;
 #pragma unroll
-      for (int j = 0; j < 14; ++j) {
+      for (int j = 0; j < NJ; ++j) {
         const int idx = lane + 64 * j;
+        if ((NH + NC + NG) % 64 != 0 && idx >= NH + NC + NG) break;
         const f32x4 v = *(const f32x4*)(sv + idx * 16);
-        if (idx < 128) {
+        if (idx < NH) {
           const int row = idx >> 3, cc = idx & 7;
           if (n0 + row < a.N)
             *(f32x4*)(a.h[d] + ((unsigned)((n0 + row) * a.P + a.padl + t) * (unsigned)a.ld_h + (unsigned)(u0 + cc * 8))) = v;
-        } else if (idx < 384) {
-          const int jj = idx - 128, row = jj >> 4, cc = jj & 15;
+        } else if (idx < NH + NC) {
+          const int jj = idx - NH, row = jj >> 4, cc = jj & 15;
           if (n0 + row < a.N)
             *(f32x4*)(a.c[d] + ((unsigned)((n0 + row) * a.P + a.padl + t) * (unsigned)H + (unsigned)(u0 + cc * 4))) = v;
         } else {
-          const int jj = idx - 384, row = jj >> 5, gate = (jj >> 3) & 3, cc = jj & 7;
+          const int jj = idx - NH - NC, row = jj >> 5, gate = (jj >> 3) & 3, cc = jj & 7;
           if (n0 + row < a.N)
             *(f32x4*)(a.gates[d] + ((unsigned)((n0 + row) * a.P + a.padl + t) * (unsigned)(4 * H) + (unsigned)(gate * H + u0 + cc * 8))) = v;
         }
@@ -537,15 +545,15 @@
     wg_barrier();
     save(Q - 1);
   } else {
-    f32x4 pf[16];
+    f32x4 pf[RPC];
     const float* xg = a.xg[d];
     const int pgate = lane >> 4, pf4 = (lane & 15) * 4;
     auto pf_load = [&](int q) {
       const int step = q / R, rg = q % R;
       const int t = d ? T - 1 - step : step;
-      const int n0 = (rg0 + rg) * 16;
-#pragma unroll
-      for (int j = 0; j < 16; ++j) {
+      const int n0 = (rg0 + rg) * RPC;
+#pragma unroll
+      for (int j = 0; j < RPC; ++j) {
         const int n = n0 + j;
         pf[j] = n < a.N ? *(const f32x4*)(xg + ((unsigned)(n * a.P + a.padl + t) * (unsigned)a.ld_xg + (unsigned)(pgate * H + u0 + pf4)))
                         : (f32x4){0.f, 0.f, 0.f, 0.f};
@@ -553,7 +561,7 @@
     };
     auto pf_store = [&](int buf) {
 #pragma unroll
-      for (int j = 0; j < 16; ++j) *(f32x4*)(xgs + ((size_t)buf * 16 + j) * XG_LD + pgate * 64 + pf4) = pf[j];
+      for (int j = 0; j < RPC; ++j) *(f32x4*)(xgs + ((size_t)buf * 16 + j) * XG_LD + pgate * 64 + pf4) = pf[j];
     };
     pf_load(0);
     pf_store(0);
@@ -576,23 +584,24 @@
 constexpr int X3_WAVES = X3W + X3_POLL + 2;
 constexpr int XG3_LD = 4 * X3_UPW + 4;
 
-template <int HB, int R>
+template <int HB, int R, int RPC>
 __global__ __launch_bounds__(X3_WAVES * 64) void lstm_cluster3_fwd_kernel(LstmClusterArgs a) {
   extern __shared__ __attribute__((aligned(16))) char smem[];
-  constexpr int H = HB * 64, KS = H / 32, GPC = 16 * H;
+  static_assert(RPC == 16 || ((RPC == 8 || RPC == 4) && R == 1), "rows per chain");
+  constexpr int H = HB * 64, KS = H / 32, GPC = RPC * H;
   constexpr int CS = H / X3_UPW;
   constexpr int PPG = GPC / (X3_POLL * 64);
   static_assert(GPC % (X3_POLL * 64) == 0, "poller coverage");
   bf16_t* hsh = (bf16_t*)smem;
   bf16_t* hsl = hsh + 2 * 16 * H;
   float* xgs = (float*)(hsl + 2 * 16 * H);
-  constexpr int SV_H = 16 * 32 * 4, SV_C = 16 * 32 * 4, SV_G = 16 * 4 * 32 * 2, SV_HB = 16 * 32 * 2;
+  constexpr int SV_H = RPC * 32 * 4, SV_C = RPC * 32 * 4, SV_G = RPC * 4 * 32 * 2, SV_HB = RPC * 32 * 2;
   constexpr int SV_BYTES = SV_H + SV_C + SV_G + SV_HB;
   char* svs = (char*)(xgs + 2 * 16 * XG3_LD);
   int* abortf = (int*)(svs + 2 * SV_BYTES);
   const int tid = threadIdx.x, lane = tid & 63;
   const int wave = __builtin_amdgcn_readfirstlane(tid >> 6);
-  const int nsets = ((a.N + 15) / 16 + R - 1) / R;
+  const int nsets = ((a.N + RPC - 1) / RPC + R - 1) / R;
   const int set = blockIdx.x / CS, wgc = blockIdx.x % CS;
   const int d = set / nsets, rg0 = (set % nsets) * R;
   const int r16 = lane & 15, g = lane >> 4;
@@ -600,11 +609,15 @@
   const int u0 = wgc * X3_UPW;
   const int T = a.T, Q = a.T * R;
   if (tid < 2) abortf[tid] = 0;
+  if (RPC < 16) {
+    for (int i = tid; i < 2 * 2 * 16 * H / 8; i += X3_WAVES * 64) ((uint4*)hsh)[i] = make_uint4(0u, 0u, 0u, 0u);
+    if (blockIdx.x == 0 && tid == 0) a.status[1] = RPC;
+  }
 
   if (wave < X3W) {
     const int ul = wave * 8 + (r16 & 7);
-    const bool cell_lane = r16 < 8;
-    const int pub0 = (((wgc * X3W + wave) * 32) + g * 8 + (r16 & 7)) * 4;
+    const bool cell_lane = r16 < 8 && (RPC == 16 || g < RPC / 4);
+    const int pub0 = (wgc * X3W + wave) * 8 * RPC + (g * 8 + (r16 & 7)) * 4;
     bf16x8 bwh[2][KS], bwl[2][KS];
     {
 #pragma unroll
@@ -624,9 +637,9 @@
     for (int rg = 0; rg < R; ++rg)
 #pragma unroll
       for (int r = 0; r < 4; ++r) {
-        const int n = (rg0 + rg) * 16 + g * 4 + r;
+        const int n = (rg0 + rg) * RPC + g * 4 + r;
         cst[rg][r] = 0.f;
-        len[rg][r] = (a.lengths && n < a.N) ? a.lengths[n] : T;
+        len[rg][r] = (a.lengths && (RPC == 16 || g < RPC / 4) && n < a.N) ? a.lengths[n] : T;
       }
     for (int step = 0; step < T; ++step) {
       const int t = d ? T - 1 - step : step;
@@ -717,9 +730,9 @@
         bf16_t* dl_ = hsl + (size_t)buf * 16 * H;
 #pragma unroll
         for (int j = 0; j < PPG; ++j) {
-          const int jj = j0 + j;
-          const int row = (((jj & 1) << 1) | pgl) * 4 + pr_;
-          const int k = (jj >> 3) * X3_UPW + ((jj >> 1) & 3) * 8 + pu;
+          const int xi = 2 * (j0 + j) + pgl;
+          const int row = (xi % (RPC / 4)) * 4 + pr_;
+          const int k = (xi / RPC) * X3_UPW + ((xi / (RPC / 4)) & 3) * 8 + pu;
           const float x = __uint_as_float((unsigned)v[j]);
           const bf16_t hi = (bf16_t)x;
           const int so = swz_off(row, k, H);
@@ -732,29 +745,31 @@
     }
     wg_barrier();
   } else if (wave == X3W + X3_POLL) {
+    constexpr int NH = RPC * 8, NG = RPC * 16, NB = RPC * 4, NJ = (2 * NH + NG + NB + 63) / 64;
     auto save = [&](int q) {
       const int step = q / R, rg = q % R;
       const int t = d ? T - 1 - step : step;
-      const int n0 = (rg0 + rg) * 16;
+      const int n0 = (rg0 + rg) * RPC;
       const char* sv = svs + (size_t)(q & 1) * SV_BYTES;
 #pragma unroll
-      for (int j = 0; j < 9; ++j) {
+      for (int j = 0; j < NJ; ++j) {
         const int idx = lane + 64 * j;
+        if ((2 * NH + NG + NB) % 64 != 0 && idx >= 2 * NH + NG + NB) break;
         const f32x4 v = *(const f32x4*)(sv + idx * 16);
-        if (idx < 128) {
+        if (idx < NH) {
           const int row = idx >> 3, cc = idx & 7;
           if (n0 + row < a.N)
             *(f32x4*)(a.hf[d] + ((unsigned)((n0 + row) * a.P + a.padl + t) * (unsigned)a.ld_h + (unsigned)(u0 + cc * 4))) = v;
-        } else if (idx < 256) {
-          const int jj = idx - 128, row = jj >> 3, cc = jj & 7;
+        } else if (idx < 2 * NH) {
+          const int jj = idx - NH, row = jj >> 3, cc = jj & 7;
           if (n0 + row < a.N)
             *(f32x4*)(a.c[d] + ((unsigned)((n0 + row) * a.P + a.padl + t) * (unsigned)H + (unsigned)(u0 + cc * 4))) = v;
-        } else if (idx < 512) {
-          const int jj = idx - 256, row = jj >> 4, gate = (jj >> 2) & 3, cc = jj & 3;
+        } else if (idx < 2 * NH + NG) {
+          const int jj = idx - 2 * NH, row = jj >> 4, gate = (jj >> 2) & 3, cc = jj & 3;
           if (n0 + row < a.N)
             *(f32x4*)(a.gates[d] + ((unsigned)((n0 + row) * a.P + a.padl + t) * (unsigned)(4 * H) + (unsigned)(gate * H + u0 + cc * 8))) = v;
         } else {
-          const int jj = idx - 512, row = jj >> 2, cc = jj & 3;
+          const int jj = idx - 2 * NH - NG, row = jj >> 2, cc = jj & 3;
           if (a.hb[d] && n0 + row < a.N)
             *(f32x4*)(a.hb[d] + ((unsigned)((n0 + row) * a.P + a.padl + t) * (unsigned)a.ld_hb + (unsigned)(u0 + cc * 8))) = v;
         }
@@ -768,15 +783,15 @@
     wg_barrier();
     save(Q - 1);
   } else {
-    f32x4 pf[8];
+    f32x4 pf[RPC / 2];
     const float* xg = a.xg[d];
     const int prow = lane >> 5, pgate = (lane >> 3) & 3, pf4 = (lane & 7) * 4;
     auto pf_load = [&](int q) {
       const int step = q / R, rg = q % R;
       const int t = d ? T - 1 - step : step;
-      const int n0 = (rg0 + rg) * 16;
-#pragma unroll
-      for (int j = 0; j < 8; ++j) {
+      const int n0 = (rg0 + rg) * RPC;
+#pragma unroll
+      for (int j = 0; j < RPC / 2; ++j) {
         const int n = n0 + 2 * j + prow;
         pf[j] = n < a.N ? *(const f32x4*)(xg + ((unsigned)(n * a.P + a.padl + t) * (unsigned)a.ld_xg + (unsigned)(pgate * H + u0 + pf4)))
                         : (f32x4){0.f, 0.f, 0.f, 0.f};
@@ -784,7 +799,7 @@
     };
     auto pf_store = [&](int buf) {
 #pragma unroll
-      for (int j = 0; j < 8; ++j) *(f32x4*)(xgs + ((size_t)buf * 16 + 2 * j + prow) * XG3_LD + pgate * X3_UPW + pf4) = pf[j];
+      for (int j = 0; j < RPC / 2; ++j) *(f32x4*)(xgs + ((size_t)buf * 16 + 2 * j + prow) * XG3_LD + pgate * X3_UPW + pf4) = pf[j];
     };
     pf_load(0);
     pf_store(0);
@@ -1041,11 +1056,12 @@
 constexpr int BP_WAVES = XW + 2;
 constexpr int DGI_LD = 256 + 8;
 
-template <int HB, int R>
+template <int HB, int R, int RPC>
 __global__ __launch_bounds__(BP_WAVES * 64) void lstm_cluster2p_bwd_kernel(LstmClusterArgs a) {
   extern __shared__ __attribute__((aligned(16))) char smem[];
   constexpr int H = HB * 64, K4 = 4 * H, CS = HB;
-  constexpr int GPD = 16 * 32;
+  static_assert(RPC == 16 || ((RPC == 8 || RPC == 4) && R == 1), "rows per chain");
+  constexpr int GPD = RPC * 32;
   bf16_t* dgi = (bf16_t*)smem;
   char* ops = (char*)(dgi + 2 * 16 * DGI_LD);
   constexpr int OPS_G = 16 * 4 * 64 * 2, OPS_F = 16 * 64 * 4;
@@ -1054,7 +1070,7 @@
   int* abortf = (int*)(c0 + R * 16 * 64);
   const int tid = threadIdx.x, lane = tid & 63;
   const int wave = __builtin_amdgcn_readfirstlane(tid >> 6);
-  const int nsets = ((a.N + 15) / 16 + R - 1) / R;
+  const int nsets = ((a.N + RPC - 1) / RPC + R - 1) / R;
   const int set = blockIdx.x / CS, wgc = blockIdx.x % CS;
   const int d = set / nsets, rg0 = (set % nsets) * R;
   const int r16 = lane & 15, g = lane >> 4;
@@ -1062,10 +1078,12 @@
   const int u0 = wgc * 64;
   const int T = a.T, Q = a.T * R;
   if (tid == 0) abortf[0] = 0;
+  if (RPC < 16 && blockIdx.x == 0 && tid == 0) a.status[1] = RPC;
   auto t_of = [&](int step) { return d ? T - 1 - step : step; };
 
   if (wave < XW) {
     const int wu = wave * 16 + r16;
+    const bool live = RPC == 16 || g < RPC / 4;
     bf16x8 bw[HB][8];
 #pragma unroll
     for (int j = 0; j < HB; ++j) {
@@ -1083,9 +1101,9 @@
       ownp[rg] = (f32x4){0.f, 0.f, 0.f, 0.f};
 #pragma unroll
       for (int r = 0; r < 4; ++r) {
-        const int n = (rg0 + rg) * 16 + g * 4 + r;
+        const int n = (rg0 + rg) * RPC + g * 4 + r;
         dcc[rg][r] = 0.f; pc[rg][r] = 0.f;
-        len[rg][r] = (a.lengths && n < a.N) ? a.lengths[n] : T;
+        len[rg][r] = (a.lengths && live && n < a.N) ? a.lengths[n] : T;
       }
     }
     float kdo[4], kdc[4], ki[4], kj[4], kf[4], dhx[4], cpv[4], gfv[4];
@@ -1120,11 +1138,11 @@
 #pragma unroll
       for (int rg = 0; rg < R; ++rg) {
         const int q = bs * R + rg, buf = q & 1;
-        const int n0 = (rg0 + rg) * 16;
+        const int n0 = (rg0 + rg) * RPC;
         const bool tr = (a.dbg & 16) && blockIdx.x == 0 && tid == 0 && q < 512;
         if (tr) a.trace[q * 8 + 0] = wall_clock64();
         f32x4 rec = ownp[rg];
-        if (bs > 0 && CS > 1) {
+        if (bs > 0 && CS > 1 && live) {
           const u64* cur = xb0 + ((size_t)rg * 2 + (bs & 1)) * CS * CS * GPD + (size_t)wgc * CS * GPD + (g * 2) * 64 + wu;
           u64 v[CS > 1 ? CS - 1 : 1][2];
           unsigned spins = 0, clk0 = 0;
@@ -1166,7 +1184,7 @@
           const float dc = dh * kdc[r] + dcc[rg][r];
           float dgv[4] = {dc * ki[r], dc * kj[r], dc * kf[r], d_o};
           dcc[rg][r] = dc * gfv[r];
-          if (t >= len[rg][r] || n >= a.N) {
+          if (t >= len[rg][r] || n >= a.N || !live) {
             dgv[0] = dgv[1] = dgv[2] = dgv[3] = 0.f;
             dcc[rg][r] = 0.f;
           }
@@ -1197,7 +1215,7 @@
           for (int j = 0; j < HB; ++j) {
             if (j == wgc) {
               ownp[rg] = acc[j];
-            } else {
+            } else if (live) {
               u64* dst = nxt + (size_t)(j * CS + wgc) * GPD + (g * 2) * 64 + wu;
 #pragma unroll
               for (int h = 0; h < 2; ++h)
@@ -1215,15 +1233,15 @@
     auto save = [&](int q) {
       const int bs = q / R, rg = q % R;
       const int t = t_of(T - 1 - bs);
-      const int n0 = (rg0 + rg) * 16;
+      const int n0 = (rg0 + rg) * RPC;
       const bf16_t* di = dgi + (size_t)(q & 1) * 16 * DGI_LD;
 #pragma unroll
-      for (int jj = 0; jj < 2; ++jj) {
+      for (int jj = 0; jj < (RPC * 8 + 63) / 64; ++jj) {
         const int idx = lane + 64 * jj, c8 = idx & 7, row = idx >> 3;
         uint2 x[8];
 #pragma unroll
         for (int e = 0; e < 8; ++e) x[e] = *(const uint2*)(di + row * DGI_LD + (c8 * 8 + e) * 4);
-        if (n0 + row < a.N) {
+        if ((RPC == 16 || row < RPC) && n0 + row < a.N) {
           bf16_t* out = a.dgates[d] + ((unsigned)((n0 + row) * a.P + a.padl + t) * (unsigned)K4 + (unsigned)(u0 + c8 * 8));
 #pragma unroll
           for (int gate = 0; gate < 4; ++gate) {
@@ -1246,21 +1264,21 @@
     }
     save(Q - 1);
   } else {
-    f32x4 pg[8], pd[4], pcp[4];
+    f32x4 pg[RPC / 2], pd[RPC / 4], pcp[RPC / 4];
     auto pf_load = [&](int q) {
       const int bs = q / R, rg = q % R, step = T - 1 - bs;
       const int t = t_of(step), tp = d ? t + 1 : t - 1;
       const bool has_prev = step > 0;
-      const int n0 = (rg0 + rg) * 16;
-#pragma unroll
-      for (int j = 0; j < 8; ++j) {
+      const int n0 = (rg0 + rg) * RPC;
+#pragma unroll
+      for (int j = 0; j < RPC / 2; ++j) {
         const int idx = lane + 64 * j, c8 = idx & 7, gate = (idx >> 3) & 3, row = idx >> 5;
         const int n = n0 + row;
         pg[j] = n < a.N ? *(const f32x4*)(a.gates[d] + ((unsigned)(n * a.P + a.padl + t) * (unsigned)(4 * H) + (unsigned)(gate * H + u0 + c8 * 8)))
                         : (f32x4){0.f, 0.f, 0.f, 0.f};
       }
 #pragma unroll
-      for (int j = 0; j < 4; ++j) {
+      for (int j = 0; j < RPC / 4; ++j) {
         const int idx = lane + 64 * j, c16 = idx & 15, row = idx >> 4;
         const int n = n0 + row;
         pd[j] = n < a.N ? *(const f32x4*)(a.dh[d] + ((unsigned)(n * a.P + a.padl + t) * (unsigned)a.ld_dh + (unsigned)(u0 + c16 * 4)))
@@ -1272,9 +1290,9 @@
     auto pf_store = [&](int buf) {
       char* st = ops + (size_t)buf * OPS_STAGE;
 #pragma unroll
-      for (int j = 0; j < 8; ++j) *(f32x4*)(st + (size_t)(lane + 64 * j) * 16) = pg[j];
-#pragma unroll
-      for (int j = 0; j < 4; ++j) {
+      for (int j = 0; j < RPC / 2; ++j) *(f32x4*)(st + (size_t)(lane + 64 * j) * 16) = pg[j];
+#pragma unroll
+      for (int j = 0; j < RPC / 4; ++j) {
         *(f32x4*)(st + OPS_G + (size_t)(lane + 64 * j) * 16) = pd[j];
         *(f32x4*)(st + OPS_G + OPS_F + (size_t)(lane + 64 * j) * 16) = pcp[j];
       }
@@ -1284,9 +1302,9 @@
 #pragma unroll
       for (int rg = 0; rg < R; ++rg)
 #pragma unroll
-        for (int j = 0; j < 4; ++j) {
+        for (int j = 0; j < RPC / 4; ++j) {
           const int idx = lane + 64 * j, c16 = idx & 15, row = idx >> 4;
-          const int n = (rg0 + rg) * 16 + row;
+          const int n = (rg0 + rg) * RPC + row;
           const f32x4 v = n < a.N ? *(const f32x4*)(a.c[d] + ((unsigned)(n * a.P + a.padl + t0) * (unsigned)H + (unsigned)(u0 + c16 * 4)))
                                   : (f32x4){0.f, 0.f, 0.f, 0.f};
           *(f32x4*)(c0 + (rg * 16 * 64) + idx * 4) = v;
@@ -1377,6 +1395,22 @@
   return true;
 }
 
+static int cluster_rows(int N, int wgs_per_chain, bool interleaved) {
+  if (interleaved) return 16;
+  const int cus = ns_device_cus();
+  auto grid = [&](int rows) { return 2 * ((N + rows - 1) / rows) * wgs_per_chain; };
+  const char* e = getenv("NS_CLUSTER_ROWS");
+  const int want = e ? atoi(e) : 0;
+  if (want == 16 || want == 8 || want == 4) {
+    int rows = want;
+    while (rows < 16 && grid(rows) > cus) rows *= 2;
+    return rows;
+  }
+  for (int rows = 4; rows < 16; rows *= 2)
+    if (grid(rows) <= cus / 2) return rows;
+  return 16;
+}
+
 extern "C" int ns_lstm_cluster_fwd(const ns_lstm_seq_params* p0, const ns_lstm_seq_params* p1, void* work,
                                    ns_stream_t s_) {
   hipStream_t s = (hipStream_t)s_;
@@ -1390,20 +1424,25 @@
     LstmClusterArgs a = {};
     fill(a, p0, p1, work);
     const int nrg = (a.N + 15) / 16, R = (nrg >= 2 && (a.dbg & 1024)) ? 2 : 1;
-    const size_t xbytes = (2 * (size_t)nrg + 2) * 2 * 16 * (size_t)a.H * sizeof(u64);
+    const int RPC = cluster_rows(a.N, a.H / X3_UPW, R == 2), nch = (a.N + RPC - 1) / RPC;
+    const size_t xbytes = (2 * (size_t)nch + 2) * 2 * RPC * (size_t)a.H * sizeof(u64);
     { const int zrc = ns_zero_async(work, ((256 + FLAG_BYTES + xbytes) + 15) & ~(size_t)15, s); if (zrc) return zrc; }
     const size_t lds3 = (size_t)2 * 2 * 16 * a.H * 2 + sizeof(float) * 2 * 16 * XG3_LD + 2 * 9216 + 32;
-    const dim3 grid((unsigned)(2 * ((nrg + R - 1) / R) * (a.H / X3_UPW))), block(X3_WAVES * 64);
+    const dim3 grid((unsigned)(2 * ((nch + R - 1) / R) * (a.H / X3_UPW))), block(X3_WAVES * 64);
 #define NS_LAUNCH_F3(HB_) \
     do { \
       static bool attr3 = false; \
       if (!attr3) { \
-        (void)hipFuncSetAttribute((const void*)lstm_cluster3_fwd_kernel<HB_, 2>, hipFuncAttributeMaxDynamicSharedMemorySize, 160 * 1024); \
-        (void)hipFuncSetAttribute((const void*)lstm_cluster3_fwd_kernel<HB_, 1>, hipFuncAttributeMaxDynamicSharedMemorySize, 160 * 1024); \
+        (void)hipFuncSetAttribute((const void*)lstm_cluster3_fwd_kernel<HB_, 2, 16>, hipFuncAttributeMaxDynamicSharedMemorySize, 160 * 1024); \
+        (void)hipFuncSetAttribute((const void*)lstm_cluster3_fwd_kernel<HB_, 1, 16>, hipFuncAttributeMaxDynamicSharedMemorySize, 160 * 1024); \
+        (void)hipFuncSetAttribute((const void*)lstm_cluster3_fwd_kernel<HB_, 1, 8>, hipFuncAttributeMaxDynamicSharedMemorySize, 160 * 1024); \
+        (void)hipFuncSetAttribute((const void*)lstm_cluster3_fwd_kernel<HB_, 1, 4>, hipFuncAttributeMaxDynamicSharedMemorySize, 160 * 1024); \
         attr3 = true; \
       } \
-      if (R == 2) hipLaunchKernelGGL((lstm_cluster3_fwd_kernel<HB_, 2>), grid, block, lds3, s, a); \
-      else hipLaunchKernelGGL((lstm_cluster3_fwd_kernel<HB_, 1>), grid, block, lds3, s, a); \
+      if (R == 2) hipLaunchKernelGGL((lstm_cluster3_fwd_kernel<HB_, 2, 16>), grid, block, lds3, s, a); \
+      else if (RPC == 8) hipLaunchKernelGGL((lstm_cluster3_fwd_kernel<HB_, 1, 8>), grid, block, lds3, s, a); \
+      else if (RPC == 4) hipLaunchKernelGGL((lstm_cluster3_fwd_kernel<HB_, 1, 4>), grid, block, lds3, s, a); \
+      else hipLaunchKernelGGL((lstm_cluster3_fwd_kernel<HB_, 1, 16>), grid, block, lds3, s, a); \
     } while (0)
     switch (a.H / 64) {
       case 1: NS_LAUNCH_F3(1); break;
@@ -1419,15 +1458,19 @@
   LstmClusterArgs a = {};
   fill(a, p0, p1, work);
   const size_t chains = 2 * (size_t)((a.N + 15) / 16);
-  const size_t xbytes = (chains + 2) * 2 * 16 * (size_t)(a.H / 2) * sizeof(u64);
+  const bool split = role_split_ok(a, false);
+  const int R = ((a.N + 15) / 16 >= 2 && (a.dbg & 512)) ? 2 : 1;
+  const int RPC = split ? cluster_rows(a.N, a.CS, R == 2) : 16, nrg = (a.N + RPC - 1) / RPC;
+  const size_t xbytes = (2 * (size_t)nrg + 2) * 2 * RPC * (size_t)(a.H / 2) * sizeof(u64);
   { const int zrc = ns_zero_async(work, ((256 + FLAG_BYTES + xbytes) + 15) & ~(size_t)15, s); if (zrc) return zrc; }
-  if (role_split_ok(a, false)) {
+  if (split) {
     const size_t lds2 = (size_t)2 * 16 * a.H * 2 + sizeof(float) * 2 * 16 * XG_LD + 2 * (2048 + 4096 + 8192) + 32;
-    const int nrg = (a.N + 15) / 16, R = (nrg >= 2 && (a.dbg & 512)) ? 2 : 1;
     const dim3 grid((unsigned)(2 * ((nrg + R - 1) / R) * a.CS)), block(FW_WAVES * 64);
 #define NS_LAUNCH_F(HB_) \
-    if (R == 2) hipLaunchKernelGGL((lstm_cluster2_fwd_kernel<HB_, 2>), grid, block, lds2, s, a); \
-    else hipLaunchKernelGGL((lstm_cluster2_fwd_kernel<HB_, 1>), grid, block, lds2, s, a)
+    if (R == 2) hipLaunchKernelGGL((lstm_cluster2_fwd_kernel<HB_, 2, 16>), grid, block, lds2, s, a); \
+    else if (RPC == 8) hipLaunchKernelGGL((lstm_cluster2_fwd_kernel<HB_, 1, 8>), grid, block, lds2, s, a); \
+    else if (RPC == 4) hipLaunchKernelGGL((lstm_cluster2_fwd_kernel<HB_, 1, 4>), grid, block, lds2, s, a); \
+    else hipLaunchKernelGGL((lstm_cluster2_fwd_kernel<HB_, 1, 16>), grid, block, lds2, s, a)
     switch (a.H / 64) {
       case 1: NS_LAUNCH_F(1); break;
       case 2: NS_LAUNCH_F(2); break;
@@ -1454,8 +1497,11 @@
   LstmClusterArgs a = {};
   fill(a, p0, p1, work);
   const size_t chains = 2 * (size_t)((a.N + 15) / 16);
+  const bool psum = role_split_ok(a, true) && !(a.dbg & 64);
+  const int RP = ((a.N + 15) / 16 >= 2 && (a.dbg & 2048)) ? 2 : 1;
+  const int RPC = psum ? cluster_rows(a.N, a.CS, RP == 2) : 16, nch = (a.N + RPC - 1) / RPC;
   const size_t xbytes = role_split_ok(a, true)
-                            ? ((a.dbg & 64) ? 0 : (chains + 2) * 2 * (size_t)a.CS * a.CS * 512 * sizeof(u64))
+                            ? ((a.dbg & 64) ? 0 : (2 * (size_t)nch + 2) * 2 * (size_t)a.CS * a.CS * RPC * 32 * sizeof(u64))
                             : (chains + 2) * 2 * 16 * (size_t)(4 * a.H / 2) * sizeof(u64);
   { const int zrc = ns_zero_async(work, ((256 + FLAG_BYTES + xbytes) + 15) & ~(size_t)15, s); if (zrc) return zrc; }
   static bool attr = false;
@@ -1468,15 +1514,17 @@
     (void)hipFuncSetAttribute((const void*)lstm_cluster2_bwd_kernel<4, 2>, hipFuncAttributeMaxDynamicSharedMemorySize, 160 * 1024);
     attr = true;
   }
-  if (role_split_ok(a, true) && !(a.dbg & 64)) {
-    const int nrg = (a.N + 15) / 16, R = (nrg >= 2 && (a.dbg & 2048)) ? 2 : 1;
+  if (psum) {
+    const int nrg = nch, R = RP;
     const int CS = a.CS;
     const size_t ldsp = (size_t)2 * 16 * DGI_LD * 2 + 2 * 16384 + sizeof(float) * (size_t)R * 16 * 64 + 32;
     const dim3 grid((unsigned)(2 * ((nrg + R - 1) / R) * CS)), block(BP_WAVES * 64);
 #define NS_LAUNCH_BP(HB_) \
     do { \
-      if (R == 2) hipLaunchKernelGGL((lstm_cluster2p_bwd_kernel<HB_, 2>), grid, block, ldsp, s, a); \
-      else hipLaunchKernelGGL((lstm_cluster2p_bwd_kernel<HB_, 1>), grid, block, ldsp, s, a); \
+      if (R == 2) hipLaunchKernelGGL((lstm_cluster2p_bwd_kernel<HB_, 2, 16>), grid, block, ldsp, s, a); \
+      else if (RPC == 8) hipLaunchKernelGGL((lstm_cluster2p_bwd_kernel<HB_, 1, 8>), grid, block, ldsp, s, a); \
+      else if (RPC == 4) hipLaunchKernelGGL((lstm_cluster2p_bwd_kernel<HB_, 1, 4>), grid, block, ldsp, s, a); \
+      else hipLaunchKernelGGL((lstm_cluster2p_bwd_kernel<HB_, 1, 16>), grid, block, ldsp, s, a); \
     } while (0)
     switch (a.H / 64) {
       case 1: NS_LAUNCH_BP(1); break;
```

Result: faster. 1.667 million mel-frames/s, median of 6 (+4.8%).
